# xiaoxiaokuye/CODLAD

Measured on NVIDIA B200. Metric: backmapped residues/sec (100-step, 10-ensemble), higher is better.
Workload: dtype f16 (tcgen05, fp32 accumulate)

## Files before the change

### codlad_b200/csrc/capi.cu

```cuda
#include <stdarg.h>
#include <string.h>

#include <map>
#include <string>
#include <vector>

#include "../../include/codlad_b200.h"
#include "decode.h"
#include "model.h"

namespace cb2 {

static thread_local char g_err[1024] = "";

void set_error(const char* fmt, ...) {
    va_list ap;
    va_start(ap, fmt);
    vsnprintf(g_err, sizeof(g_err), fmt, ap);
    va_end(ap);
}

float* plan_P(Plan& p, int which) { return p.P + (size_t)which * p.NB * p.L * 256; }

namespace {

struct TensorTable {
    std::map<std::string, const cb2_tensor*> by_name;
    TensorTable(const cb2_tensor* t, int n) {
        for (int i = 0; i < n; ++i) by_name[t[i].name] = &t[i];
    }
    const float* get(const std::string& name, long long numel) const {
        auto it = by_name.find(name);
        if (it == by_name.end()) { set_error("missing tensor '%s'", name.c_str()); return nullptr; }
        if (it->second->numel != numel) {
            set_error("tensor '%s': numel %lld, expected %lld", name.c_str(), it->second->numel, numel);
            return nullptr;
        }
        return it->second->data;
    }
};

struct Packer {
    std::vector<float> buf;
    size_t reserve(size_t n) {
        size_t off = (buf.size() + 63) & ~(size_t)63;
        buf.resize(off + n, 0.0f);
        return off;
    }
    size_t transposed(const float* W, int out, int in_total, int col0, int ncols, float scale = 1.0f) {
        size_t off = reserve((size_t)ncols * out);
        for (int k = 0; k < ncols; ++k)
            for (int o = 0; o < out; ++o) buf[off + (size_t)k * out + o] = scale * W[(size_t)o * in_total + col0 + k];
        return off;
    }
    size_t copy(const float* v, size_t n) {
        size_t off = reserve(n);
        memcpy(&buf[off], v, n * sizeof(float));
        return off;
    }
};

struct HalfPacker {
    std::vector<__half> buf;
    size_t block(const float* W, int in_total, int col0, float scale = 1.0f) {
        size_t off = buf.size();
        buf.resize(off + 128 * 128);
        for (int o = 0; o < 128; ++o)
            for (int k = 0; k < 128; ++k) buf[off + (size_t)o * 128 + k] = __float2half_rn(scale * W[(size_t)o * in_total + col0 + k]);
        return off;
    }
};

#define GET(var, name, numel)                               \
    const float* var = tt.get(name, (long long)(numel));    \
    if (!var) return 1;

template <typename T>
int dev_alloc(std::vector<void*>& owned, T** ptr, size_t count) {
    void* q = nullptr;
    CB2_CUDA(cudaMalloc(&q, count * sizeof(T) > 0 ? count * sizeof(T) : 16));
    owned.push_back(q);
    *ptr = reinterpret_cast<T*>(q);
    return 0;
}

}
}

using namespace cb2;

struct cb2_denoiser { DenoiserModel m; };
struct cb2_vae { VaeModel v; };
struct cb2_plan {
    Plan p;
    float* ca_full = nullptr;
    int *csr_row = nullptr, *csr_col = nullptr;
    int E = 0;
    signed char* orders = nullptr;
    int* slot_atom = nullptr;
    long long* out_off = nullptr;
    float *edge_w = nullptr, *S40 = nullptr, *phi = nullptr, *ic = nullptr, *zq = nullptr;
    int* vq_idx = nullptr;
    float *xa = nullptr, *xb = nullptr;
    int keep_debug = 0;
    bool frames_ready = false, topo_ready = false;
};

extern "C" {

int cb2_abi_version(void) { return CB2_ABI_VERSION; }
const char* cb2_last_error(void) { return cb2::g_err; }

int cb2_denoiser_create(const cb2_tensor* tensors, int n_tensors, const float* freqs128, int k_neighbors, cb2_denoiser** out) {
    if (!tensors || !freqs128 || !out) { set_error("denoiser_create: null argument"); return 1; }
    TensorTable tt(tensors, n_tensors);
    Packer pk;
    HalfPacker bp;
    const int H = CB2_H;
    std::map<std::string, size_t> off;
    std::map<std::string, size_t> boff;

    off["freqs"] = pk.copy(freqs128, 128);
    GET(te0w, "t_embedder.mlp.0.weight", H * 256) GET(te0b, "t_embedder.mlp.0.bias", H)
    GET(te2w, "t_embedder.mlp.2.weight", H * H) GET(te2b, "t_embedder.mlp.2.bias", H)
    off["te_w0_t"] = pk.transposed(te0w, H, 256, 0, 256); off["te_b0"] = pk.copy(te0b, H);
    off["te_w2_t"] = pk.transposed(te2w, H, H, 0, H); off["te_b2"] = pk.copy(te2b, H);

    {
        size_t wo = pk.reserve((size_t)H * CB2_MOD_TOTAL), bo = pk.reserve(CB2_MOD_TOTAL);
        off["ada_w_t"] = wo; off["ada_b"] = bo;
        int col = 0;
        auto put = [&](const std::string& pre, int width) -> int {
            const float* w = tt.get(pre + ".adaLN_modulation.1.weight", (long long)width * H);
            const float* b = tt.get(pre + ".adaLN_modulation.1.bias", width);
            if (!w || !b) return 1;
            for (int o = 0; o < width; ++o) {
                pk.buf[bo + col + o] = b[o];
                for (int k = 0; k < H; ++k) pk.buf[wo + (size_t)k * CB2_MOD_TOTAL + col + o] = w[(size_t)o * H + k];
            }
            col += width;
            return 0;
        };
        for (int l = 0; l < 3; ++l) if (put("encoder_layers." + std::to_string(l), CB2_MOD_ENC)) return 1;
        for (int l = 0; l < 3; ++l) if (put("decoder_layers." + std::to_string(l), CB2_MOD_DEC)) return 1;
        if (put("W_out", CB2_MOD_FIN)) return 1;
    }
    GET(xinw, "x_in.weight", H * 3) GET(xinb, "x_in.bias", H)
    off["xin_w_t"] = pk.transposed(xinw, H, 3, 0, 3); off["xin_b"] = pk.copy(xinb, H);

    GET(posw, "features.embeddings.linear.weight", 16 * 66) GET(posb, "features.embeddings.linear.bias", 16)
    GET(edgew, "features.edge_embedding.weight", H * 167)
    GET(lnw, "features.norm_edges.weight", H) GET(lnb, "features.norm_edges.bias", H)
    GET(wew, "W_e.weight", H * H) GET(web, "W_e.bias", H)
    {
        size_t o = pk.reserve(65 * H);
        for (int d = 0; d < 65; ++d)
            for (int c = 0; c < H; ++c) {
                double a = 0.0;
                for (int q = 0; q < 16; ++q) a += (double)(posw[q * 66 + d] + posb[q]) * (double)edgew[(size_t)c * 167 + q];
                pk.buf[o + (size_t)d * H + c] = (float)a;
            }
        off["pos_table"] = o;
        size_t w = pk.reserve(152 * H);
        for (int r = 0; r < 151; ++r)
            for (int c = 0; c < H; ++c) pk.buf[w + (size_t)r * H + c] = edgew[(size_t)c * 167 + 16 + r];
        off["wedge_t"] = w;
    }
    off["ln_w"] = pk.copy(lnw, H); off["ln_b"] = pk.copy(lnb, H);
    off["we_t"] = pk.transposed(wew, H, H, 0, H); off["we_b"] = pk.copy(web, H);

    GET(ws, "W_s.weight", 30 * H)
    for (int l = 0; l < 3; ++l) {
        const std::string p = "encoder_layers." + std::to_string(l), k = "e" + std::to_string(l) + ".";
        GET(w1, p + ".W1.weight", H * 3 * H) GET(b1, p + ".W1.bias", H) GET(w2, p + ".W2.weight", H * H) GET(b2, p + ".W2.bias", H)
        GET(w3, p + ".W3.weight", H * H) GET(b3, p + ".W3.bias", H)
        GET(w11, p + ".W11.weight", H * 3 * H) GET(b11, p + ".W11.bias", H) GET(w12, p + ".W12.weight", H * H) GET(b12, p + ".W12.bias", H)
        GET(w13, p + ".W13.weight", H * H) GET(b13, p + ".W13.bias", H)
        GET(win, p + ".dense.W_in.weight", 4 * H * H) GET(bin, p + ".dense.W_in.bias", 4 * H)
        GET(wout, p + ".dense.W_out.weight", H * 4 * H) GET(bout, p + ".dense.W_out.bias", H)
        off[k + "W1a_t"] = pk.transposed(w1, H, 3 * H, 0, H); off[k + "W1b_t"] = pk.transposed(w1, H, 3 * H, H, H);
        off[k + "W1c_t"] = pk.transposed(w1, H, 3 * H, 2 * H, H); off[k + "b1"] = pk.copy(b1, H);
        off[k + "W2_t"] = pk.transposed(w2, H, H, 0, H); off[k + "b2"] = pk.copy(b2, H);
        off[k + "W3_t"] = pk.transposed(w3, H, H, 0, H); off[k + "b3"] = pk.copy(b3, H);
        off[k + "W11a_t"] = pk.transposed(w11, H, 3 * H, 0, H); off[k + "W11b_t"] = pk.transposed(w11, H, 3 * H, H, H);
        off[k + "W11c_t"] = pk.transposed(w11, H, 3 * H, 2 * H, H); off[k + "b11"] = pk.copy(b11, H);
        off[k + "W12_t"] = pk.transposed(w12, H, H, 0, H); off[k + "b12"] = pk.copy(b12, H);
        off[k + "W13_t"] = pk.transposed(w13, H, H, 0, H); off[k + "b13"] = pk.copy(b13, H);
        off[k + "Win_t"] = pk.transposed(win, 4 * H, H, 0, H); off[k + "bin"] = pk.copy(bin, 4 * H);
        off[k + "Wout_t"] = pk.transposed(wout, H, 4 * H, 0, 4 * H); off[k + "bout"] = pk.copy(bout, H);
        boff[k + "W1b"] = bp.block(w1, 3 * H, H); boff[k + "W2"] = bp.block(w2, H, 0, 0.5f);
        boff[k + "W11b"] = bp.block(w11, 3 * H, H); boff[k + "W12"] = bp.block(w12, H, 0, 0.5f); boff[k + "W13"] = bp.block(w13, H, 0, 0.5f);
        boff[k + "W1a"] = bp.block(w1, 3 * H, 0); boff[k + "W1c"] = bp.block(w1, 3 * H, 2 * H);
        boff[k + "W11a"] = bp.block(w11, 3 * H, 0); boff[k + "W11c"] = bp.block(w11, 3 * H, 2 * H);
        boff[k + "W3"] = bp.block(w3, H, 0);
        for (int q = 0; q < 4; ++q) { size_t o = bp.block(win + (size_t)q * H * H, H, 0); if (q == 0) boff[k + "Win"] = o; }
        for (int q = 0; q < 4; ++q) { size_t o = bp.block(wout, 4 * H, q * H, 0.5f); if (q == 0) boff[k + "Wout"] = o; }
    }
    for (int l = 0; l < 3; ++l) {
        const std::string p = "decoder_layers." + std::to_string(l), k = "d" + std::to_string(l) + ".";
        GET(w1, p + ".W1.weight", H * 4 * H) GET(b1, p + ".W1.bias", H) GET(w2, p + ".W2.weight", H * H) GET(b2, p + ".W2.bias", H)
        GET(w3, p + ".W3.weight", H * H) GET(b3, p + ".W3.bias", H)
        GET(win, p + ".dense.W_in.weight", 4 * H * H) GET(bin, p + ".dense.W_in.bias", 4 * H)
        GET(wout, p + ".dense.W_out.weight", H * 4 * H) GET(bout, p + ".dense.W_out.bias", H)
        off[k + "W1a_t"] = pk.transposed(w1, H, 4 * H, 0, H); off[k + "W1b2_t"] = pk.transposed(w1, H, 4 * H, H, H, 2.0f);
        off[k + "W1d_t"] = pk.transposed(w1, H, 4 * H, 3 * H, H); off[k + "b1"] = pk.copy(b1, H);
        {
            size_t o = pk.reserve(30 * H);
            for (int z = 0; z < 30; ++z)
                for (int c = 0; c < H; ++c) {
                    double a = 0.0;
                    for (int q = 0; q < H; ++q) a += (double)ws[z * H + q] * (double)w1[(size_t)c * 4 * H + 2 * H + q];
                    pk.buf[o + (size_t)z * H + c] = (float)(2.0 * a);
                }
            off[k + "TS"] = o;
        }
        off[k + "W2_t"] = pk.transposed(w2, H, H, 0, H); off[k + "b2"] = pk.copy(b2, H);
        off[k + "W3_t"] = pk.transposed(w3, H, H, 0, H); off[k + "b3"] = pk.copy(b3, H);
        off[k + "Win_t"] = pk.transposed(win, 4 * H, H, 0, H); off[k + "bin"] = pk.copy(bin, 4 * H);
        off[k + "Wout_t"] = pk.transposed(wout, H, 4 * H, 0, 4 * H); off[k + "bout"] = pk.copy(bout, H);
        boff[k + "W1b2"] = bp.block(w1, 4 * H, H, 2.0f); boff[k + "W2"] = bp.block(w2, H, 0, 0.5f);
        boff[k + "W1a"] = bp.block(w1, 4 * H, 0); boff[k + "W1d"] = bp.block(w1, 4 * H, 3 * H);
        boff[k + "W3"] = bp.block(w3, H, 0);
        for (int q = 0; q < 4; ++q) { size_t o = bp.block(win + (size_t)q * H * H, H, 0); if (q == 0) boff[k + "Win"] = o; }
        for (int q = 0; q < 4; ++q) { size_t o = bp.block(wout, 4 * H, q * H, 0.5f); if (q == 0) boff[k + "Wout"] = o; }
    }
    GET(finw, "W_out.linear.weight", 6 * H) GET(finb, "W_out.linear.bias", 6)
    off["fin_w_t"] = pk.transposed(finw, 6, H, 0, H); off["fin_b"] = pk.copy(finb, 6);

    cb2_denoiser* d = new cb2_denoiser();
    DenoiserModel& m = d->m;
    m.k_neighbors = k_neighbors;
    CB2_CUDA(cudaMalloc(&m.dev_f32, pk.buf.size() * sizeof(float)));
    CB2_CUDA(cudaMemcpy(m.dev_f32, pk.buf.data(), pk.buf.size() * sizeof(float), cudaMemcpyHostToDevice));
    {
        std::vector<__half> v16;
        std::map<std::string, size_t> voff;
        auto putv = [&](const std::string& key, const float* src) {
            voff[key] = v16.size();
            for (int q = 0; q < H; ++q) v16.push_back(__float2half_rn(src[q]));
        };
        for (int l = 0; l < 3; ++l) {
            const std::string pe = "encoder_layers." + std::to_string(l), pd = "decoder_layers." + std::to_string(l);
            putv("e" + std::to_string(l) + ".b2", tt.get(pe + ".W2.bias", H));
            putv("e" + std::to_string(l) + ".b12", tt.get(pe + ".W12.bias", H));
            putv("e" + std::to_string(l) + ".b13", tt.get(pe + ".W13.bias", H));
            putv("d" + std::to_string(l) + ".b2", tt.get(pd + ".W2.bias", H));
        }
        CB2_CUDA(cudaMalloc(&m.dev_vec16, v16.size() * sizeof(__half)));
        CB2_CUDA(cudaMemcpy(m.dev_vec16, v16.data(), v16.size() * sizeof(__half), cudaMemcpyHostToDevice));
        for (int l = 0; l < 3; ++l) {
            m.enc[l].b2_16 = m.dev_vec16 + voff.at("e" + std::to_string(l) + ".b2");
            m.enc[l].b12_16 = m.dev_vec16 + voff.at("e" + std::to_string(l) + ".b12");
            m.enc[l].b13_16 = m.dev_vec16 + voff.at("e" + std::to_string(l) + ".b13");
            m.dec[l].b2_16 = m.dev_vec16 + voff.at("d" + std::to_string(l) + ".b2");
        }
    }
    CB2_CUDA(cudaMalloc(&m.dev_f16, bp.buf.size() * sizeof(__half)));
    CB2_CUDA(cudaMemcpy(m.dev_f16, bp.buf.data(), bp.buf.size() * sizeof(__half), cudaMemcpyHostToDevice));
    m.n_f16_blocks = (int)(bp.buf.size() / (128 * 128));
    auto F = [&](const std::string& key) { return (const float*)(m.dev_f32 + off.at(key)); };
    auto B = [&](const std::string& key) { return (const __half*)(m.dev_f16 + boff.at(key)); };
    m.freqs = F("freqs"); m.te_w0_t = F("te_w0_t"); m.te_b0 = F("te_b0"); m.te_w2_t = F("te_w2_t"); m.te_b2 = F("te_b2");
    m.ada_w_t = F("ada_w_t"); m.ada_b = F("ada_b"); m.xin_w_t = F("xin_w_t"); m.xin_b = F("xin_b");
    m.pos_table = F("pos_table"); m.wedge_t = F("wedge_t"); m.ln_w = F("ln_w"); m.ln_b = F("ln_b"); m.we_t = F("we_t"); m.we_b = F("we_b");
    for (int l = 0; l < 3; ++l) {
        const std::string k = "e" + std::to_string(l) + ".";
        EncLayerW& e = m.enc[l];
        e.W1a_t = F(k + "W1a_t"); e.W1b_t = F(k + "W1b_t"); e.W1c_t = F(k + "W1c_t"); e.b1 = F(k + "b1");
        e.W2_t = F(k + "W2_t"); e.b2 = F(k + "b2"); e.W3_t = F(k + "W3_t"); e.b3 = F(k + "b3");
        e.W11a_t = F(k + "W11a_t"); e.W11b_t = F(k + "W11b_t"); e.W11c_t = F(k + "W11c_t"); e.b11 = F(k + "b11");
        e.W12_t = F(k + "W12_t"); e.b12 = F(k + "b12"); e.W13_t = F(k + "W13_t"); e.b13 = F(k + "b13");
        e.Win_t = F(k + "Win_t"); e.bin = F(k + "bin"); e.Wout_t = F(k + "Wout_t"); e.bout = F(k + "bout");
        e.W1b_h = B(k + "W1b"); e.W2_h = B(k + "W2"); e.W11b_h = B(k + "W11b"); e.W12_h = B(k + "W12"); e.W13_h = B(k + "W13");
        e.W1a_h = B(k + "W1a"); e.W1c_h = B(k + "W1c"); e.W11a_h = B(k + "W11a"); e.W11c_h = B(k + "W11c");
        e.W3_h = B(k + "W3"); e.Win_h = B(k + "Win"); e.Wout_h = B(k + "Wout");
    }
    for (int l = 0; l < 3; ++l) {
        const std::string k = "d" + std::to_string(l) + ".";
        DecLayerW& e = m.dec[l];
        e.W1a_t = F(k + "W1a_t"); e.W1b2_t = F(k + "W1b2_t"); e.W1d_t = F(k + "W1d_t"); e.b1 = F(k + "b1"); e.TS = F(k + "TS");
        e.W2_t = F(k + "W2_t"); e.b2 = F(k + "b2"); e.W3_t = F(k + "W3_t"); e.b3 = F(k + "b3");
        e.Win_t = F(k + "Win_t"); e.bin = F(k + "bin"); e.Wout_t = F(k + "Wout_t"); e.bout = F(k + "bout");
        e.W1b2_h = B(k + "W1b2"); e.W2_h = B(k + "W2");
        e.W1a_h = B(k + "W1a"); e.W1d_h = B(k + "W1d"); e.W3_h = B(k + "W3"); e.Win_h = B(k + "Win"); e.Wout_h = B(k + "Wout");
    }
    m.fin_w_t = F("fin_w_t"); m.fin_b = F("fin_b");
    *out = d;
    return 0;
}

void cb2_denoiser_destroy(cb2_denoiser* d) {
    if (!d) return;
    cudaFree(d->m.dev_f32);
    cudaFree(d->m.dev_f16);
    cudaFree(d->m.dev_vec16);
    delete d;
}

int cb2_vae_create(const cb2_tensor* tensors, int n_tensors, const float* mean3, const float* std3, int angle_variant, cb2_vae** out) {
    if (!tensors || !mean3 || !std3 || !out) { set_error("vae_create: null argument"); return 1; }
    TensorTable tt(tensors, n_tensors);
    Packer pk;
    std::map<std::string, size_t> off;
    const std::string P = "equivaraintconv.";
    auto itcb = tt.by_name.find("quantize._codebook.embed");
    if (itcb == tt.by_name.end() || itcb->second->numel % 3 != 0) { set_error("missing/invalid quantize._codebook.embed"); return 1; }
    const int M = (int)(itcb->second->numel / 3);
    off["codebook"] = pk.copy(itcb->second->data, (size_t)M * 3);
    off["mean"] = pk.copy(mean3, 3); off["std"] = pk.copy(std3, 3);
    GET(mow, "map_out.weight", 36 * 3) GET(mob, "map_out.bias", 36)
    off["mapw_t"] = pk.transposed(mow, 36, 3, 0, 3); off["mapb"] = pk.copy(mob, 36);
    GET(remb, P + "res_embed.weight", 25 * 4) off["res_embed"] = pk.copy(remb, 100);
    const int D = 40, T = angle_variant ? 50 : 40;
    auto linear = [&](const std::string& key, const std::string& name, int o, int i) -> int {
        const float* w = tt.get(P + name + ".weight", (long long)o * i);
        const float* b = tt.get(P + name + ".bias", o);
        if (!w || !b) return 1;
        off[key + "_t"] = pk.transposed(w, o, i, 0, i);
        off[key + "_b"] = pk.copy(b, o);
        return 0;
    };
    size_t wd = pk.reserve(4 * 15 * D), bd = pk.reserve(4 * D);
    off["Wd_t"] = wd; off["bd"] = bd;
    for (int b = 0; b < 4; ++b) {
        const std::string s = std::to_string(b);
        if (linear("inv0." + s, "message_blocks." + s + ".inv_dense.0", D, D)) return 1;
        if (linear("inv1." + s, "message_blocks." + s + ".inv_dense.1", D, D)) return 1;
        GET(dw, P + "message_blocks." + s + ".dist_embed.block.1.weight", D * 15)
        GET(db, P + "message_blocks." + s + ".dist_embed.block.1.bias", D)
        for (int q = 0; q < 15; ++q)
            for (int c = 0; c < D; ++c) pk.buf[wd + ((size_t)b * 15 + q) * D + c] = dw[c * 15 + q];
        for (int c = 0; c < D; ++c) pk.buf[bd + b * D + c] = db[c];
        if (linear("db1." + s, "dense_blocks." + s + ".1", D, D)) return 1;
        if (linear("db3." + s, "dense_blocks." + s + ".3", D, D)) return 1;
        if (linear("tb1." + s, "sidechain_torsion_blocks." + s + ".1", T, T)) return 1;
        if (linear("tb3." + s, "sidechain_torsion_blocks." + s + ".3", T, T)) return 1;
    }
    GET(bbd, P + "backbone_dist.weight", 75) GET(scd, P + "sidechain_dist.weight", 250)
    off["bb_dist"] = pk.copy(bbd, 75); off["sc_dist"] = pk.copy(scd, 250);
    if (linear("ba1", "backbone_angle.1", 3, D) || linear("ba3", "backbone_angle.3", 3, 3)) return 1;
    if (linear("bt1", "backbone_torsion.1", 3, D + 3) || linear("bt3", "backbone_torsion.3", 3, 3)) return 1;
    if (angle_variant) {
        if (linear("sa1", "sidechain_angle.1", 10, D) || linear("sa3", "sidechain_angle.3", 10, 10)) return 1;
    } else {
        GET(sae, P + "sidechain_angle.weight", 250) off["sa_embed"] = pk.copy(sae, 250);
    }
    if (linear("ft1", "final_torsion.1", 10, T) || linear("ft3", "final_torsion.3", 10, 10)) return 1;

    cb2_vae* h = new cb2_vae();
    VaeModel& v = h->v;
    v.M = M; v.angle_variant = angle_variant;
    CB2_CUDA(cudaMalloc(&v.dev, pk.buf.size() * sizeof(float)));
    CB2_CUDA(cudaMemcpy(v.dev, pk.buf.data(), pk.buf.size() * sizeof(float), cudaMemcpyHostToDevice));
    auto F = [&](const std::string& key) -> const float* {
        auto it = off.find(key);
        return it == off.end() ? nullptr : (const float*)(v.dev + it->second);
    };
    v.codebook = F("codebook"); v.mean = F("mean"); v.stdv = F("std"); v.mapw_t = F("mapw_t"); v.mapb = F("mapb");
    v.res_embed = F("res_embed"); v.Wd_t = F("Wd_t"); v.bd = F("bd");
    for (int b = 0; b < 4; ++b) {
        const std::string s = std::to_string(b);
        v.inv0_t[b] = F("inv0." + s + "_t"); v.inv0_b[b] = F("inv0." + s + "_b");
        v.inv1_t[b] = F("inv1." + s + "_t"); v.inv1_b[b] = F("inv1." + s + "_b");
        v.db1_t[b] = F("db1." + s + "_t"); v.db1_b[b] = F("db1." + s + "_b");
        v.db3_t[b] = F("db3." + s + "_t"); v.db3_b[b] = F("db3." + s + "_b");
        v.tb1_t[b] = F("tb1." + s + "_t"); v.tb1_b[b] = F("tb1." + s + "_b");
        v.tb3_t[b] = F("tb3." + s + "_t"); v.tb3_b[b] = F("tb3." + s + "_b");
    }
    v.bb_dist = F("bb_dist"); v.sc_dist = F("sc_dist"); v.sa_embed = F("sa_embed");
    v.ba1_t = F("ba1_t"); v.ba1_b = F("ba1_b"); v.ba3_t = F("ba3_t"); v.ba3_b = F("ba3_b");
    v.bt1_t = F("bt1_t"); v.bt1_b = F("bt1_b"); v.bt3_t = F("bt3_t"); v.bt3_b = F("bt3_b");
    v.sa1_t = F("sa1_t"); v.sa1_b = F("sa1_b"); v.sa3_t = F("sa3_t"); v.sa3_b = F("sa3_b");
    v.ft1_t = F("ft1_t"); v.ft1_b = F("ft1_b"); v.ft3_t = F("ft3_t"); v.ft3_b = F("ft3_b");
    CB2_CUDA(cudaMalloc(&v.e2, (size_t)M * sizeof(float)));
    if (int e = launch_codebook_norms(v.codebook, M, v.e2, 0)) return e;
    CB2_CUDA(cudaStreamSynchronize(0));
    *out = h;
    return 0;
}

void cb2_vae_destroy(cb2_vae* h) {
    if (!h) return;
    cudaFree(h->v.dev);
    cudaFree(h->v.e2);
    delete h;
}

int cb2_plan_create(const cb2_denoiser* d, int F, int NB, int L, int precision, int keep_debug, cb2_plan** out) {
    if (!out || F <= 0 || NB <= 0 || L <= 0) { set_error("plan_create: bad argument"); return 1; }
    if (precision != PREC_F32 && precision != PREC_F16) { set_error("plan_create: unknown precision %d", precision); return 1; }
    cb2_plan* h = new cb2_plan();
    Plan& p = h->p;
    p.model = d ? &d->m : nullptr; p.F = F; p.NB = NB; p.L = L; p.precision = precision;
    h->keep_debug = keep_debug;
    if (!d) {
        int e = 0;
        e |= dev_alloc(p.allocs, &p.X, (size_t)F * L * 3);
        e |= dev_alloc(p.allocs, &p.lengths, F);
        e |= dev_alloc(p.allocs, &p.cg_z, (size_t)F * L);
        e |= dev_alloc(p.allocs, &p.frame_of, NB);
        if (e) { cb2_plan_destroy(h); return e; }
        *out = h;
        return 0;
    }
    p.K = d->m.k_neighbors < L ? d->m.k_neighbors : L;
    const size_t N = (size_t)NB * L, FE = (size_t)F * L * p.K, NE = N * p.K;
    const size_t esz = precision == PREC_F16 ? 2 : 4;
    int e = 0;
    e |= dev_alloc(p.allocs, &p.X, (size_t)F * L * 3);
    e |= dev_alloc(p.allocs, &p.lengths, F);
    e |= dev_alloc(p.allocs, &p.cg_z, (size_t)F * L);
    e |= dev_alloc(p.allocs, &p.frame_of, NB);
    e |= dev_alloc(p.allocs, &p.nbr_idx, FE);
    e |= dev_alloc(p.allocs, &p.nbr_dist, FE);
    e |= dev_alloc(p.allocs, reinterpret_cast<unsigned char**>(&p.hE0), FE * 128 * esz);
    e |= dev_alloc(p.allocs, reinterpret_cast<unsigned char**>(&p.hE), NE * 128 * esz);
    if (keep_debug) e |= dev_alloc(p.allocs, &p.E_dbg, FE * 128);
    e |= dev_alloc(p.allocs, &p.hV, N * 128);
    e |= dev_alloc(p.allocs, &p.hVenc, N * 128);
    e |= dev_alloc(p.allocs, &p.P, 2 * N * 256);
    if (precision == PREC_F16) {
        e |= dev_alloc(p.allocs, &p.P16[0], N * 256);
        e |= dev_alloc(p.allocs, &p.P16[1], N * 256);
    }
    e |= dev_alloc(p.allocs, &p.S, N * 128);
    e |= dev_alloc(p.allocs, &p.out6, N * 6);
    e |= dev_alloc(p.allocs, &h->xa, N * 3);
    e |= dev_alloc(p.allocs, &h->xb, N * 3);
    p.mod_capacity = NB > 1024 ? NB : 1024;
    e |= dev_alloc(p.allocs, &p.mod, (size_t)p.mod_capacity * CB2_MOD_TOTAL);
    if (precision == PREC_F16) e |= dev_alloc(p.allocs, &p.mod16, (size_t)p.mod_capacity * 768);
    e |= dev_alloc(p.allocs, &p.silu_c, (size_t)p.mod_capacity * 128);
    e |= dev_alloc(p.allocs, &p.tvals, p.mod_capacity);
    e |= dev_alloc(p.allocs, &p.coef, (size_t)p.mod_capacity * 8);
    if (e) { cb2_plan_destroy(h); return e; }
    if (precision == PREC_F16) {
        if (int r = edge_tc_prepare(p)) { cb2_plan_destroy(h); return r; }
        if (int r = node_tc_prepare(p)) { cb2_plan_destroy(h); return r; }
    }
    *out = h;
    return 0;
}

void cb2_plan_destroy(cb2_plan* h) {
    if (!h) return;
    if (h->p.graph) cudaGraphExecDestroy(h->p.graph);
    edge_tc_release(h->p);
    node_tc_release(h->p);
    for (void* q : h->p.allocs) cudaFree(q);
    delete h;
}

int cb2_plan_K(const cb2_plan* h) { return h ? h->p.K : 0; }
long long cb2_plan_launches(const cb2_plan* h) { return h ? h->p.launches : 0; }

int cb2_plan_set_frames(cb2_plan* h, const float* X, const int* lengths, const int* cg_z, const int* frame_of, void* stream) {
    if (!h || !X || !lengths || !cg_z || !frame_of) { set_error("set_frames: null argument"); return 1; }
    Plan& p = h->p;
    cudaStream_t s = (cudaStream_t)stream;
    CB2_CUDA(cudaMemcpyAsync(p.X, X, (size_t)p.F * p.L * 3 * sizeof(float), cudaMemcpyDeviceToDevice, s));
    CB2_CUDA(cudaMemcpyAsync(p.lengths, lengths, p.F * sizeof(int), cudaMemcpyDeviceToDevice, s));
    CB2_CUDA(cudaMemcpyAsync(p.cg_z, cg_z, (size_t)p.F * p.L * sizeof(int), cudaMemcpyDeviceToDevice, s));
    CB2_CUDA(cudaMemcpyAsync(p.frame_of, frame_of, p.NB * sizeof(int), cudaMemcpyDeviceToDevice, s));
    if (p.model == nullptr) { h->frames_ready = true; return 0; }
    {
        std::vector<int> len((size_t)p.F);
        CB2_CUDA(cudaMemcpyAsync(len.data(), p.lengths, (size_t)p.F * sizeof(int), cudaMemcpyDeviceToHost, s));
        CB2_CUDA(cudaStreamSynchronize(s));
        p.all_full = true;
        for (int f = 0; f < p.F; ++f) p.all_full = p.all_full && len[f] >= p.L;
    }
    if (int e = launch_knn(p.X, p.lengths, p.F, p.L, p.K, p.nbr_dist, p.nbr_idx, s)) return e;
    if (int e = launch_edge_features(*p.model, p.X, p.lengths, p.nbr_idx, p.nbr_dist, p.F, p.L, p.K, p.E_dbg, p.hE0, p.precision, s)) return e;
    p.launches += 2;
    h->frames_ready = true;
    return 0;
}

}

namespace {

int edge_dispatch(Plan& p, int mode, int layer, const float* mod_base, int mod_stride, cudaStream_t s) {
    return p.precision == PREC_F16 ? launch_edge_tc(p, mode, layer, mod_base, mod_stride, s)
                                    : launch_edge_f32(p, mode, layer, mod_base, mod_stride, s);
}

int run_forward(Plan& p, const float* x, const float* mod_base, int mod_stride, const float* noise, float* x_next,
                const float* coef_row, const float* inpaint_row, cudaStream_t s, int stop_after = -1) {
    int n = 0;
    auto done = [&]() { return stop_after >= 0 && ++n >= stop_after; };
    const bool tc = p.precision == PREC_F16 && p.node_tc != nullptr;
    auto node_update = [&](int phase, const float* xt, const float* nz, float* xn, const float* cf, const float* iq) {
        return tc ? launch_node_update_tc(p, phase, mod_base, mod_stride, xt, nz, xn, cf, iq, s)
                  : launch_node_update(p, phase, mod_base, mod_stride, xt, nz, xn, cf, iq, s);
    };
    if (int e = tc ? launch_node_init_tc(p, x, s) : launch_node_init(p, x, mod_base, mod_stride, s)) return e;
    if (done()) return 0;
    for (int l = 0; l < 3; ++l) {
        if (int e = edge_dispatch(p, EDGE_ENC_NODE, l, mod_base, mod_stride, s)) return e;
        if (done()) return 0;
        if (int e = node_update(l, nullptr, nullptr, nullptr, nullptr, nullptr)) return e;
        if (done()) return 0;
        if (int e = edge_dispatch(p, EDGE_ENC_EDGE, l, mod_base, mod_stride, s)) return e;
        if (done()) return 0;
    }
    for (int l = 0; l < 3; ++l) {
        if (int e = edge_dispatch(p, EDGE_DEC, l, mod_base, mod_stride, s)) return e;
        if (done()) return 0;
        const bool last = l == 2;
        if (int e = node_update(3 + l, last ? x : nullptr, last ? noise : nullptr, last ? x_next : nullptr, last ? coef_row : nullptr,
                                last ? inpaint_row : nullptr)) return e;
        if (done()) return 0;
    }
    return 0;
}

}

extern "C" {

int cb2_plan_forward_partial(cb2_plan* h, const float* x, const float* t, int stop_after, void* stream) {
    if (!h || !x || !t) { set_error("forward_partial: null argument"); return 1; }
    if (!h->frames_ready || !h->p.model) { set_error("forward_partial: no denoiser frames on this plan"); return 1; }
    Plan& p = h->p;
    cudaStream_t s = (cudaStream_t)stream;
    if (int e = launch_timestep_mod(*p.model, t, p.NB, p.silu_c, p.mod, p.mod16, s)) return e;
    p.coef_steps = 0;
    return run_forward(p, x, p.mod, CB2_MOD_TOTAL, nullptr, nullptr, nullptr, nullptr, s, stop_after);
}

int cb2_plan_forward(cb2_plan* h, const float* x, const float* t, float* out, void* stream) {
    if (!h || !x || !t || !out) { set_error("forward: null argument"); return 1; }
    if (!h->frames_ready || !h->p.model) { set_error("forward: cb2_plan_set_frames has not been called (or decode-only plan)"); return 1; }
    Plan& p = h->p;
    cudaStream_t s = (cudaStream_t)stream;
    if (p.NB > p.mod_capacity) { set_error("forward: NB exceeds table capacity"); return 1; }
    if (int e = launch_timestep_mod(*p.model, t, p.NB, p.silu_c, p.mod, p.mod16, s)) return e;
    p.launches += 2;
    p.coef_steps = 0;
    if (int e = run_forward(p, x, p.mod, CB2_MOD_TOTAL, nullptr, nullptr, nullptr, nullptr, s)) return e;
    CB2_CUDA(cudaMemcpyAsync(out, p.out6, (size_t)p.NB * p.L * 6 * sizeof(float), cudaMemcpyDeviceToDevice, s));
    return 0;
}

static int set_schedule(cb2_plan* h, const float* t_of_step, const float* coef, int T, int kind, cudaStream_t s) {
    if (!h || !t_of_step || !coef || T <= 0 || !h->p.model) { set_error("set_schedule: bad argument"); return 1; }
    Plan& p = h->p;
    if (T > p.mod_capacity) { set_error("set_schedule: T=%d exceeds capacity %d", T, p.mod_capacity); return 1; }
    CB2_CUDA(cudaMemcpyAsync(p.tvals, t_of_step, T * sizeof(float), cudaMemcpyHostToDevice, s));
    CB2_CUDA(cudaMemcpyAsync(p.coef, coef, (size_t)T * 8 * sizeof(float), cudaMemcpyHostToDevice, s));
    if (int e = launch_timestep_mod(*p.model, p.tvals, T, p.silu_c, p.mod, p.mod16, s)) return e;
    CB2_CUDA(cudaStreamSynchronize(s));
    p.launches += 2;
    p.coef_steps = T;
    p.update_kind = kind;
    p.coef_noisy = kind == UPDATE_DDPM;
    for (int i = 0; i < T && !p.coef_noisy; ++i) p.coef_noisy = coef[(size_t)i * 8 + 4] != 0.0f;
    if (p.graph) { cudaGraphExecDestroy(p.graph); p.graph = nullptr; }
    return 0;
}

int cb2_plan_set_schedule(cb2_plan* h, const float* t_of_step, const float* coef, int T, void* stream) {
    return set_schedule(h, t_of_step, coef, T, UPDATE_DDPM, (cudaStream_t)stream);
}

int cb2_plan_set_ddim_schedule(cb2_plan* h, const float* t_of_step, const float* ddim_coef, int T, void* stream) {
    return set_schedule(h, t_of_step, ddim_coef, T, UPDATE_DDIM, (cudaStream_t)stream);
}

int cb2_plan_set_inpaint(cb2_plan* h, const unsigned char* keep, const float* x0, const float* q_coef, int T, void* stream) {
    if (!h || !h->p.model) { set_error("set_inpaint: bad argument"); return 1; }
    Plan& p = h->p;
    if (!keep) { p.inpaint = false; return 0; }
    if (!x0 || !q_coef || T <= 0) { set_error("set_inpaint: x0, q_coef and T > 0 are required with a keep mask"); return 1; }
    if (T > p.mod_capacity) { set_error("set_inpaint: T=%d exceeds capacity %d", T, p.mod_capacity); return 1; }
    cudaStream_t s = (cudaStream_t)stream;
    const size_t N = (size_t)p.NB * p.L;
    if (!p.inp_keep) {
        unsigned char* keep_buf = nullptr;
        float *x0_buf = nullptr, *eps_buf = nullptr, *coef_buf = nullptr;
        int e = 0;
        e |= dev_alloc(p.allocs, &keep_buf, N);
        e |= dev_alloc(p.allocs, &x0_buf, N * 3);
        e |= dev_alloc(p.allocs, &eps_buf, N * 3);
        e |= dev_alloc(p.allocs, &coef_buf, (size_t)(p.mod_capacity + 1) * 2);
        if (e) return e;
        p.inp_keep = keep_buf; p.inp_x0 = x0_buf; p.inp_eps = eps_buf; p.inp_coef = coef_buf;
    }
    CB2_CUDA(cudaMemcpyAsync(p.inp_keep, keep, N, cudaMemcpyDeviceToDevice, s));
    CB2_CUDA(cudaMemcpyAsync(p.inp_x0, x0, N * 3 * sizeof(float), cudaMemcpyDeviceToDevice, s));
    const size_t nq = (size_t)(T + 1) * 2;
    if (p.inp_coef_host.size() != nq || memcmp(p.inp_coef_host.data(), q_coef, nq * sizeof(float)) != 0) {
        p.inp_coef_host.assign(q_coef, q_coef + nq);
        CB2_CUDA(cudaMemcpyAsync(p.inp_coef, q_coef, nq * sizeof(float), cudaMemcpyHostToDevice, s));
        CB2_CUDA(cudaStreamSynchronize(s));
    }
    p.inpaint_steps = T;
    p.inpaint = true;
    return 0;
}

static int enqueue_loop(cb2_plan* h, float* x, const float* noise, cudaStream_t s) {
    Plan& p = h->p;
    const size_t n3 = (size_t)p.NB * p.L * 3;
    CB2_CUDA(cudaMemcpyAsync(h->xa, x, n3 * sizeof(float), cudaMemcpyDeviceToDevice, s));
    if (p.inpaint) {
        if (int e = launch_inpaint_init(p.inp_keep, p.inp_x0, p.inp_coef + (size_t)p.coef_steps * 2, p.NB * p.L, h->xa, p.inp_eps, s)) return e;
        p.launches++;
    }
    float *cur = h->xa, *nxt = h->xb;
    for (int step = p.coef_steps - 1; step >= 0; --step) {
        const float* mod_row = p.mod + (size_t)step * CB2_MOD_TOTAL;
        const float* step_noise = noise != nullptr ? noise + (size_t)step * n3 : nullptr;
        const float* inpaint_row = p.inpaint ? p.inp_coef + (size_t)step * 2 : nullptr;
        if (int e = run_forward(p, cur, mod_row, 0, step_noise, nxt, p.coef + (size_t)step * 8, inpaint_row, s)) {
            char prev[1024];
            snprintf(prev, sizeof(prev), "%s", g_err);
            const unsigned int* tl = edge_tc_trap_log();
            if (tl != nullptr) {
                char w[600]; int n = 0;
                for (int i = 0; i < 18 && n < 560; ++i)
                    if (tl[4 + 2 * i]) n += snprintf(w + n, sizeof(w) - n, " w%d:bar+0x%x/p%u", i, tl[4 + 2 * i] & 0xfffu, tl[5 + 2 * i] >> 16);
                set_error("%s [sampling step %d; block %u timed-out waits:%s]", prev, step, tl[0] - 1u, w);
            }
            else set_error("%s [sampling step %d]", prev, step);
            return e;
        }
        float* t = cur; cur = nxt; nxt = t;
    }
    CB2_CUDA(cudaMemcpyAsync(x, cur, n3 * sizeof(float), cudaMemcpyDeviceToDevice, s));
    return 0;
}

int cb2_plan_sample(cb2_plan* h, float* x, const float* noise, int use_graph, void* stream) {
    if (!h || !x) { set_error("sample: null argument"); return 1; }
    Plan& p = h->p;
    if (!h->frames_ready || p.coef_steps <= 0) { set_error("sample: set_frames / set_schedule must be called first"); return 1; }
    if (!noise && p.coef_noisy) { set_error("sample: noise may be NULL only on a DDIM schedule whose sigma are all zero (eta = 0)"); return 1; }
    if (p.inpaint && p.inpaint_steps != p.coef_steps) {
        set_error("sample: the inpainting table has T=%d, the schedule T=%d", p.inpaint_steps, p.coef_steps);
        return 1;
    }
    cudaStream_t s = (cudaStream_t)stream;
    if (!use_graph) return enqueue_loop(h, x, noise, s);
    if (!p.graph || p.graph_key[0] != x || p.graph_key[1] != noise || p.graph_steps != p.coef_steps || p.graph_all_full != p.all_full ||
        p.graph_inpaint != p.inpaint) {
        if (p.graph) { cudaGraphExecDestroy(p.graph); p.graph = nullptr; }
        cudaStream_t cs;
        CB2_CUDA(cudaStreamCreateWithFlags(&cs, cudaStreamNonBlocking));
        const long long before = p.launches;
        CB2_CUDA(cudaStreamBeginCapture(cs, cudaStreamCaptureModeThreadLocal));
        int e = enqueue_loop(h, x, noise, cs);
        cudaGraph_t g = nullptr;
        cudaError_t ce = cudaStreamEndCapture(cs, &g);
        p.launches = before;
        if (e || ce != cudaSuccess) {
            if (g) cudaGraphDestroy(g);
            cudaStreamDestroy(cs);
            if (!e) set_error("graph capture failed: %s", cudaGetErrorString(ce));
            return e ? e : (int)ce;
        }
        ce = cudaGraphInstantiate(&p.graph, g, 0);
        cudaGraphDestroy(g);
        cudaStreamDestroy(cs);
        if (ce != cudaSuccess) { set_error("graph instantiate failed: %s", cudaGetErrorString(ce)); p.graph = nullptr; return (int)ce; }
        p.graph_key[0] = x; p.graph_key[1] = noise; p.graph_steps = p.coef_steps; p.graph_all_full = p.all_full;
        p.graph_inpaint = p.inpaint;
    }
    CB2_CUDA(cudaGraphLaunch(p.graph, s));
    p.launches += 16LL * p.coef_steps + (p.inpaint ? 1 : 0);
    return 0;
}

int cb2_plan_set_topology(cb2_plan* h, const cb2_vae* v, const float* ca_full, const int* csr_row_ptr, const int* csr_col,
                          int n_edges, const signed char* atom_orders, const int* slot_atom, const long long* out_offset,
                          void* stream) {
    if (!h || !v || !ca_full || !csr_row_ptr || !atom_orders || !slot_atom || !out_offset) { set_error("set_topology: null argument"); return 1; }
    Plan& p = h->p;
    cudaStream_t s = (cudaStream_t)stream;
    const size_t N = (size_t)p.NB * p.L, FL = (size_t)p.F * p.L;
    if (!h->ca_full) {
        int e = 0;
        e |= dev_alloc(p.allocs, &h->ca_full, (size_t)p.F * (p.L + 2) * 3);
        e |= dev_alloc(p.allocs, &h->csr_row, FL + 1);
        e |= dev_alloc(p.allocs, &h->orders, FL * 30);
        e |= dev_alloc(p.allocs, &h->slot_atom, FL * 14);
        e |= dev_alloc(p.allocs, &h->out_off, p.NB);
        e |= dev_alloc(p.allocs, &h->S40, N * 40);
        e |= dev_alloc(p.allocs, &h->phi, N * 40);
        e |= dev_alloc(p.allocs, &h->ic, N * 39);
        e |= dev_alloc(p.allocs, &h->zq, N * 3);
        e |= dev_alloc(p.allocs, &h->vq_idx, N);
        if (e) return e;
    }
    if (n_edges > h->E || !h->csr_col) {
        int e = dev_alloc(p.allocs, &h->csr_col, (size_t)n_edges);
        e |= dev_alloc(p.allocs, &h->edge_w, (size_t)4 * n_edges * 40);
        if (e) return e;
    }
    h->E = n_edges;
    CB2_CUDA(cudaMemcpyAsync(h->ca_full, ca_full, (size_t)p.F * (p.L + 2) * 3 * sizeof(float), cudaMemcpyDeviceToDevice, s));
    CB2_CUDA(cudaMemcpyAsync(h->csr_row, csr_row_ptr, (FL + 1) * sizeof(int), cudaMemcpyDefault, s));
    if (n_edges) CB2_CUDA(cudaMemcpyAsync(h->csr_col, csr_col, (size_t)n_edges * sizeof(int), cudaMemcpyDefault, s));
    CB2_CUDA(cudaMemcpyAsync(h->orders, atom_orders, FL * 30, cudaMemcpyDefault, s));
    CB2_CUDA(cudaMemcpyAsync(h->slot_atom, slot_atom, FL * 14 * sizeof(int), cudaMemcpyDefault, s));
    CB2_CUDA(cudaMemcpyAsync(h->out_off, out_offset, p.NB * sizeof(long long), cudaMemcpyDefault, s));
    if (!h->frames_ready) { set_error("set_topology: call cb2_plan_set_frames first (needs X)"); return 1; }
    if (int e = launch_ic_edge_filters(v->v, p.X, p.F, p.L, h->csr_row, h->csr_col, n_edges, h->edge_w, s)) return e;
    p.launches += 1;
    CB2_CUDA(cudaStreamSynchronize(s));
    h->topo_ready = true;
    return 0;
}

int cb2_plan_decode(cb2_plan* h, const cb2_vae* v, const float* latent, int denorm, int* idx, float* zq, float* ic_recon,
                    float* xyz, void* stream) {
    if (!h || !v || !latent) { set_error("decode: null argument"); return 1; }
    if (!h->topo_ready) { set_error("decode: cb2_plan_set_topology has not been called"); return 1; }
    Plan& p = h->p;
    cudaStream_t s = (cudaStream_t)stream;
    const int N = p.NB * p.L;
    if (int e = launch_vq_lookup(v->v, latent, N, p.L, p.lengths, p.frame_of, denorm, h->vq_idx, h->zq, h->S40, s)) return e;
    if (int e = launch_ic_decoder(v->v, h->S40, h->phi, N, p.L, p.frame_of, p.lengths, p.cg_z, h->csr_row, h->csr_col, h->E,
                                  h->edge_w, h->ic, s, &p.launches)) return e;
    p.launches += 1;
    if (idx) CB2_CUDA(cudaMemcpyAsync(idx, h->vq_idx, (size_t)N * sizeof(int), cudaMemcpyDeviceToDevice, s));
    if (zq) CB2_CUDA(cudaMemcpyAsync(zq, h->zq, (size_t)N * 3 * sizeof(float), cudaMemcpyDeviceToDevice, s));
    if (ic_recon) CB2_CUDA(cudaMemcpyAsync(ic_recon, h->ic, (size_t)N * 39 * sizeof(float), cudaMemcpyDeviceToDevice, s));
    if (xyz) {
        if (int e = launch_ic_to_xyz(h->ca_full, h->ic, N, p.L, p.frame_of, p.lengths, h->orders, h->slot_atom, h->out_off, xyz,
                                     nullptr, s)) return e;
        p.launches += 1;
    }
    return 0;
}

int cb2_plan_buffer(cb2_plan* h, const char* name, void* dst, long long dst_bytes, void* stream) {
    if (!h || !name || !dst) { set_error("plan_buffer: null argument"); return 1; }
    void* src = nullptr;
    long long size = 0;
    void** ptr = &src;
    long long* bytes = &size;
    Plan& p = h->p;
    const size_t N = (size_t)p.NB * p.L, FE = (size_t)p.F * p.L * p.K, esz = p.precision == PREC_F16 ? 2 : 4;
    const std::string n = name;
    if (n == "nbr_idx") { *ptr = p.nbr_idx; *bytes = FE * 4; }
    else if (n == "nbr_dist") { *ptr = p.nbr_dist; *bytes = FE * 4; }
    else if (n == "E") { *ptr = p.E_dbg; *bytes = p.E_dbg ? FE * 128 * 4 : 0; }
    else if (n == "hE0") { *ptr = p.hE0; *bytes = FE * 128 * esz; }
    else if (n == "hE") { *ptr = p.hE; *bytes = N * p.K * 128 * esz; }
    else if (n == "hV") { *ptr = p.hV; *bytes = N * 128 * 4; }
    else if (n == "S") { *ptr = p.S; *bytes = N * 128 * 4; }
    else if (n == "out6") { *ptr = p.out6; *bytes = N * 6 * 4; }
    else if (n == "tc_trace") {
        if (!p.tc_trace) { unsigned long long* t = nullptr; if (dev_alloc(p.allocs, &t, 6144)) return 1; cudaMemsetAsync(t, 0, 49152, (cudaStream_t)stream); p.tc_trace = t; }
        *ptr = p.tc_trace; *bytes = 49152;
    }
    else if (n == "mod") { *ptr = p.mod; *bytes = (size_t)p.mod_capacity * CB2_MOD_TOTAL * 4; }
    else { set_error("plan_buffer: unknown buffer '%s'", name); return 1; }
    if (!src || dst_bytes > size) { set_error("plan_buffer: '%s' holds %lld bytes, %lld requested", name, size, dst_bytes); return 1; }
    CB2_CUDA(cudaMemcpyAsync(dst, src, (size_t)dst_bytes, cudaMemcpyDeviceToDevice, (cudaStream_t)stream));
    return 0;
}

int cb2_plan_run_edge_kernel(cb2_plan* h, int mode, int layer, void* stream) {
    if (!h || mode < 0 || mode > 2 || layer < 0 || layer > 2) { set_error("run_edge_kernel: bad argument"); return 1; }
    if (!h->frames_ready || h->p.coef_steps <= 0) { set_error("run_edge_kernel: set_frames / set_schedule first"); return 1; }
    return edge_dispatch(h->p, mode, layer, h->p.mod, 0, (cudaStream_t)stream);
}

int cb2_plan_run_stage(cb2_plan* h, const cb2_vae* v, int stage, int layer, float* xyz_scratch, void* stream) {
    if (!h || stage < 0 || stage > 9) { set_error("run_stage: bad argument"); return 1; }
    Plan& p = h->p;
    cudaStream_t s = (cudaStream_t)stream;
    if (!h->frames_ready) { set_error("run_stage: set_frames first"); return 1; }
    if (stage <= 3 && (p.coef_steps <= 0 || !p.model)) { set_error("run_stage: set_schedule first"); return 1; }
    if (stage >= 6 && (!h->topo_ready || !v)) { set_error("run_stage: set_topology first (and pass the vae)"); return 1; }
    const int N = p.NB * p.L;
    switch (stage) {
        case 0: case 1: case 2:
            if (layer < 0 || layer > 2) { set_error("run_stage: layer"); return 1; }
            return edge_dispatch(p, stage, layer, p.mod, 0, s);
        case 3: {
            if (layer < 0 || layer > 5) { set_error("run_stage: phase"); return 1; }
            const bool last = layer == 5, tc = p.precision == PREC_F16 && p.node_tc != nullptr;
            const float *xt = last ? h->xa : nullptr, *nz = last ? h->xa : nullptr, *cf = last ? p.coef : nullptr;
            float* xn = last ? h->xb : nullptr;
            return tc ? launch_node_update_tc(p, layer, p.mod, 0, xt, nz, xn, cf, nullptr, s)
                      : launch_node_update(p, layer, p.mod, 0, xt, nz, xn, cf, nullptr, s);
        }
        case 4: return launch_knn(p.X, p.lengths, p.F, p.L, p.K, p.nbr_dist, p.nbr_idx, s);
        case 5: return launch_edge_features(*p.model, p.X, p.lengths, p.nbr_idx, p.nbr_dist, p.F, p.L, p.K, p.E_dbg, p.hE0, p.precision, s);
        case 6: return launch_vq_lookup(v->v, h->xa, N, p.L, p.lengths, p.frame_of, 1, h->vq_idx, h->zq, h->S40, s);
        case 7: return launch_ic_decoder(v->v, h->S40, h->phi, N, p.L, p.frame_of, p.lengths, p.cg_z, h->csr_row, h->csr_col, h->E, h->edge_w, h->ic, s, &p.launches);
        case 8:
            if (!xyz_scratch) { set_error("run_stage: ic_to_xyz needs xyz_scratch"); return 1; }
            return launch_ic_to_xyz(h->ca_full, h->ic, N, p.L, p.frame_of, p.lengths, h->orders, h->slot_atom, h->out_off, xyz_scratch, nullptr, s);
        default: return launch_ic_edge_filters(v->v, p.X, p.F, p.L, h->csr_row, h->csr_col, h->E, h->edge_w, s);
    }
}

int cb2_knn_topk(const float* X, const int* lengths, int F, int L, int K, float* D, int* idx, void* stream) {
    if (!X || !D || !idx) { set_error("knn_topk: null argument"); return 1; }
    return launch_knn(X, lengths, F, L, K, D, idx, (cudaStream_t)stream);
}

int cb2_vq_lookup(const cb2_vae* v, const float* x, int NB, int L, const int* lengths, const int* frame_of, int denorm,
                  int* idx, float* zq, void* stream) {
    if (!v || !x || !lengths || !frame_of || !idx || !zq) { set_error("vq_lookup: null argument"); return 1; }
    return launch_vq_lookup(v->v, x, NB * L, L, lengths, frame_of, denorm, idx, zq, nullptr, (cudaStream_t)stream);
}

int cb2_p_sample(const float* x, const float* model_out, const float* noise, const float* coef, const int* step_of_member,
                 int rows_per_member, int rows, int C, float* x_next, void* stream) {
    if (!x || !model_out || !noise || !coef || !step_of_member || !x_next) { set_error("p_sample: null argument"); return 1; }
    return launch_p_sample(x, model_out, noise, coef, step_of_member, rows_per_member, rows, C, x_next, (cudaStream_t)stream);
}

int cb2_ddim_sample(const float* x, const float* model_out, const float* noise, const float* coef, const int* step_of_member,
                    int rows_per_member, int rows, int C, float* x_next, void* stream) {
    if (!x || !model_out || !coef || !step_of_member || !x_next) { set_error("ddim_sample: null argument"); return 1; }
    return launch_ddim_sample(x, model_out, noise, coef, step_of_member, rows_per_member, rows, C, x_next, (cudaStream_t)stream);
}

int cb2_ic_to_xyz(const float* ca_full, const float* ic_recon, int NB, int L, const int* frame_of, const int* lengths,
                  const signed char* atom_orders, const int* slot_atom, const long long* out_offset, float* xyz, void* stream) {
    if (!ca_full || !ic_recon || !frame_of || !lengths || !atom_orders || !slot_atom || !out_offset || !xyz) {
        set_error("ic_to_xyz: null argument");
        return 1;
    }
    return launch_ic_to_xyz(ca_full, ic_recon, NB * L, L, frame_of, lengths, atom_orders, slot_atom, out_offset, xyz, nullptr,
                            (cudaStream_t)stream);
}

}
```

### codlad_b200/csrc/model.h

```cpp
#pragma once
#include <cuda_runtime.h>
#include <cuda_fp16.h>
#include <stdint.h>
#include <string>
#include <unordered_map>
#include <vector>

#include "common.cuh"

namespace cb2 {

struct EncLayerW {
    const float *W1a_t, *W1b_t, *W1c_t, *b1, *W2_t, *b2, *W3_t, *b3;
    const float *W11a_t, *W11b_t, *W11c_t, *b11, *W12_t, *b12, *W13_t, *b13;
    const float *Win_t, *bin, *Wout_t, *bout;
    const __half *W1b_h, *W2_h, *W11b_h, *W12_h, *W13_h;
    const __half *W1a_h, *W1c_h, *W11a_h, *W11c_h, *W3_h, *Win_h , *Wout_h ;
    const __half *b2_16, *b12_16, *b13_16;
};

struct DecLayerW {
    const float *W1a_t, *W1b2_t , *W1d_t, *b1, *TS ;
    const float *W2_t, *b2, *W3_t, *b3, *Win_t, *bin, *Wout_t, *bout;
    const __half *W1b2_h, *W2_h;
    const __half *W1a_h, *W1d_h, *W3_h, *Win_h , *Wout_h ;
    const __half* b2_16;
};

struct DenoiserModel {
    int k_neighbors = 64;
    int vocab = 30;
    const float *freqs , *te_w0_t, *te_b0, *te_w2_t, *te_b2, *ada_w_t, *ada_b;
    const float *xin_w_t , *xin_b;
    const float *pos_table, *wedge_t, *ln_w, *ln_b, *we_t, *we_b;
    EncLayerW enc[3];
    DecLayerW dec[3];
    const float *fin_w_t , *fin_b;
    float* dev_f32 = nullptr;
    __half* dev_f16 = nullptr;
    __half* dev_vec16 = nullptr;
    int n_f16_blocks = 0;
};

enum Precision { PREC_F32 = 0, PREC_F16 = 1 };
enum UpdateKind { UPDATE_DDPM = 0, UPDATE_DDIM = 1 };

struct Plan {
    const DenoiserModel* model = nullptr;
    int F = 0, NB = 0, L = 0, K = 0, precision = PREC_F32;
    int T_rows = 0;
    float* X = nullptr;
    int* lengths = nullptr;
    int* cg_z = nullptr;
    int* frame_of = nullptr;
    int* nbr_idx = nullptr;
    float* nbr_dist = nullptr;
    void* hE0 = nullptr;
    float* E_dbg = nullptr;
    void* hE = nullptr;
    float* hV = nullptr;
    float* hVenc = nullptr;
    float* P = nullptr;
    __half* P16[2] = {nullptr, nullptr};
    __half* mod16 = nullptr;
    int num_sms = 148;
    bool all_full = false;
    unsigned long long* tc_trace = nullptr;
    float* silu_c = nullptr;
    float* S = nullptr;
    float* out6 = nullptr;
    float* mod = nullptr;
    int mod_capacity = 0;
    int* mod_row = nullptr;
    float* tvals = nullptr;
    float* coef = nullptr;
    int coef_steps = 0;
    int update_kind = 0;
    bool coef_noisy = true;
    bool inpaint = false;
    int inpaint_steps = 0;
    unsigned char* inp_keep = nullptr;
    float* inp_x0 = nullptr;
    float* inp_eps = nullptr;
    float* inp_coef = nullptr;
    std::vector<float> inp_coef_host;
    cudaGraphExec_t graph = nullptr;
    const void* graph_key[4] = {nullptr, nullptr, nullptr, nullptr};
    int graph_steps = 0;
    bool graph_all_full = false;
    bool graph_inpaint = false;
    std::vector<void*> allocs;
    void* tmaps = nullptr;
    void* node_tc = nullptr;
    long long launches = 0;
};

int launch_knn(const float* X, const int* lengths, int F, int L, int K, float* D, int* idx, cudaStream_t s);
int launch_edge_features(const DenoiserModel& m, const float* X, const int* lengths, const int* idx, const float* D,
                         int F, int L, int K, float* E_dbg, void* hE0, int precision, cudaStream_t s);
int launch_edge_raw_features(const float* X, const int* idx, const float* D, int F, int L, int K, float* raw_out, cudaStream_t s);
int launch_timestep_mod(const DenoiserModel& m, const float* tvals, int n, float* scratch_silu_c, float* mod, __half* mod16, cudaStream_t s);
int launch_p_sample(const float* x, const float* out6, const float* noise, const float* coef_rows, const int* step_of_row,
                    int rows_per_b, int n_rows, int C, float* x_next, cudaStream_t s);
int launch_ddim_sample(const float* x, const float* out6, const float* noise, const float* coef_rows, const int* step_of_row,
                       int rows_per_b, int n_rows, int C, float* x_next, cudaStream_t s);
int launch_inpaint_init(const unsigned char* keep, const float* x0, const float* q_head, int n_rows, float* x, float* eps, cudaStream_t s);
float* plan_P(Plan& p, int which);

struct NodeArgs;
int launch_node_init(Plan& p, const float* x, const float* mod_base, int mod_stride_b, cudaStream_t s);
int launch_node_update(Plan& p, int phase , const float* mod_base, int mod_stride_b,
                       const float* x_t, const float* noise, float* x_next, const float* coef_row, const float* inpaint_row,
                       cudaStream_t s);
int launch_edge_f32(Plan& p, int mode, int layer, const float* mod_base, int mod_stride_b, cudaStream_t s);
int launch_edge_tc(Plan& p, int mode, int layer, const float* mod_base, int mod_stride_b, cudaStream_t s);
int edge_tc_prepare(Plan& p);
int node_tc_prepare(Plan& p);
void node_tc_release(Plan& p);
int launch_node_init_tc(Plan& p, const float* x, cudaStream_t s);
int launch_node_update_tc(Plan& p, int phase, const float* mod_base, int mod_stride_b, const float* x_t, const float* noise,
                          float* x_next, const float* coef_row, const float* inpaint_row, cudaStream_t s);
void edge_tc_release(Plan& p);
const unsigned int* edge_tc_trap_log();

enum EdgeMode { EDGE_ENC_NODE = 0, EDGE_ENC_EDGE = 1, EDGE_DEC = 2 };

}
```

### codlad_b200/csrc/node_tc.cu

```cuda
#include "node_tc_body.cuh"

namespace cb2 {

using namespace tc;

namespace {

template <bool INPAINT>
__device__ __forceinline__ void node_tc_run(const CUtensorMap& wmap, const NodeTcParams& p, const InpaintRows& ir) {
    extern __shared__ __align__(1024) unsigned char smem[];
    __shared__ uint32_t s_tmem;
    const int tid = threadIdx.x, warp = tid >> 5;
    if (tid == 0) trace_window(p.trace, p.trace_slot, false);
    if ((smem_u32(smem) & 1023u) != 0) __trap();
    pdl_launch_dependents();
    if (warp == 16) {
        asm volatile("tcgen05.alloc.cta_group::1.sync.aligned.shared::cta.b32 [%0], 512;" ::"r"(smem_u32(&s_tmem)) : "memory");
        asm volatile("tcgen05.relinquish_alloc_permit.cta_group::1.sync.aligned;" ::: "memory");
    }
    tc_fence_before();
    __syncthreads();
    tc_fence_after();
    const uint32_t tmem_base = s_tmem;
    node_block<INPAINT>(smem, tmem_base, &wmap, p, blockIdx.x * NT, p.N, true, ir);
    if (tid == 0) trace_window(p.trace, p.trace_slot, true);
    if (warp == 16) asm volatile("tcgen05.dealloc.cta_group::1.sync.aligned.b32 %0, 512;" ::"r"(tmem_base) : "memory");
}

__global__ void __launch_bounds__(NODE_CTA_THREADS, 1) node_tc_kernel(const __grid_constant__ CUtensorMap wmap, const NodeTcParams p) {
    node_tc_run<false>(wmap, p, InpaintRows{});
}

__global__ void __launch_bounds__(NODE_CTA_THREADS, 1) node_tc_inpaint_kernel(const __grid_constant__ CUtensorMap wmap, const NodeTcParams p,
                                                                             const __grid_constant__ InpaintRows ir) {
    node_tc_run<true>(wmap, p, ir);
}


struct NodeTcState { CUtensorMap wmap; };

int node_tc_launch(Plan& p, NodeTcParams& np, cudaStream_t s, const InpaintRows* ir = nullptr) {
    const NodeTcState& st = *reinterpret_cast<const NodeTcState*>(p.node_tc);
    const dim3 grid((np.N + NT - 1) / NT), block(NODE_CTA_THREADS);
    if (ir != nullptr) CB2_CUDA(launch_pdl(node_tc_inpaint_kernel, grid, block, NODE_TC_SMEM, s, st.wmap, np, *ir));
    else CB2_CUDA(launch_pdl(node_tc_kernel, grid, block, NODE_TC_SMEM, s, st.wmap, np));
    CB2_LAUNCH_CHECK();
    p.launches++;
    return 0;
}

void base_params(Plan& p, NodeTcParams& np) {
    np = NodeTcParams{};
    np.N = p.NB * p.L; np.L = p.L; np.K = p.K;
    np.lengths = p.lengths; np.frame_of = p.frame_of; np.nbr_idx = p.nbr_idx; np.cg_z = p.cg_z;
    np.hV = p.hV; np.hVenc = p.hVenc; np.S = p.S;
    np.trace = p.tc_trace; np.trace_slot = p.launches & 2047;
}

}

int node_tc_prepare(Plan& p) {
    EncodeTiledFn fn = nullptr;
    if (get_encode_fn(&fn)) return 1;
    NodeTcState* st = new NodeTcState();
    p.node_tc = st;
    if (encode_rows_map(fn, &st->wmap, p.model->dev_f16, (size_t)p.model->n_f16_blocks * 128, 128)) return 1;
    CB2_CUDA(cudaFuncSetAttribute(node_tc_kernel, cudaFuncAttributeMaxDynamicSharedMemorySize, (int)NODE_TC_SMEM));
    CB2_CUDA(cudaFuncSetAttribute(node_tc_inpaint_kernel, cudaFuncAttributeMaxDynamicSharedMemorySize, (int)NODE_TC_SMEM));
    return 0;
}

void node_tc_release(Plan& p) {
    delete reinterpret_cast<NodeTcState*>(p.node_tc);
    p.node_tc = nullptr;
}

int launch_node_init_tc(Plan& p, const float* x, cudaStream_t s) {
    const DenoiserModel& m = *p.model;
    auto row_of = [&](const __half* w) { return (int)((w - m.dev_f16) / 128); };
    NodeTcParams np;
    base_params(p, np);
    np.do_update = 0;
    np.x = x; np.xin_w_t = m.xin_w_t; np.xin_b = m.xin_b;
    np.n_proj = 1;
    np.proj[0] = ProjTc{row_of(m.enc[0].W1a_h), row_of(m.enc[0].W1c_h), m.enc[0].b1, nullptr, p.P16[0], 0};
    return node_tc_launch(p, np, s);
}

void node_tc_update_params(Plan& p, int phase, const float* mod_base, int mod_stride_b, const float* x_t, const float* noise,
                           float* x_next, const float* coef_row, tc::NodeTcParams& np) {
    const DenoiserModel& m = *p.model;
    auto row_of = [&](const __half* w) { return (int)((w - m.dev_f16) / 128); };
    base_params(p, np);
    np.do_update = 1;
    np.mod_stride = mod_stride_b;
    if (phase < 3) {
        const EncLayerW& e = m.enc[phase];
        np.masked_count = 1;
        np.w3_row = row_of(e.W3_h); np.win_row = row_of(e.Win_h); np.wout_row = row_of(e.Wout_h);
        np.b3 = e.b3; np.bin = e.bin; np.bout = e.bout;
        np.mod = mod_base + CB2_MOD_ENC_OFF(phase);
        np.n_proj = 2;
        np.proj[0] = ProjTc{row_of(e.W11a_h), row_of(e.W11c_h), e.b11, nullptr, p.P16[1], 0};
        if (phase < 2) {
            const EncLayerW& nx = m.enc[phase + 1];
            np.proj[1] = ProjTc{row_of(nx.W1a_h), row_of(nx.W1c_h), nx.b1, nullptr, p.P16[0], 0};
        } else {
            const DecLayerW& d = m.dec[0];
            np.write_enc = 1;
            np.proj[1] = ProjTc{row_of(d.W1a_h), row_of(d.W1d_h), d.b1, d.TS, p.P16[0], 2};
        }
    } else {
        const int l = phase - 3;
        const DecLayerW& d = m.dec[l];
        np.masked_count = 0;
        np.w3_row = row_of(d.W3_h); np.win_row = row_of(d.Win_h); np.wout_row = row_of(d.Wout_h);
        np.b3 = d.b3; np.bin = d.bin; np.bout = d.bout;
        np.mod = mod_base + CB2_MOD_DEC_OFF(l);
        if (l < 2) {
            const DecLayerW& nx = m.dec[l + 1];
            np.n_proj = 1;
            np.proj[0] = ProjTc{row_of(nx.W1a_h), row_of(nx.W1d_h), nx.b1, nx.TS, p.P16[0], 1};
        } else {
            np.n_proj = 0;
            np.do_final = 1;
            np.fin_mod = mod_base + CB2_MOD_FIN_OFF;
            np.fin_w_t = m.fin_w_t; np.fin_b = m.fin_b;
            np.out6 = p.out6;
            np.x_t = x_t; np.noise = noise; np.x_next = x_next; np.coef = coef_row;
            np.ddim = p.update_kind == UPDATE_DDIM;
        }
    }
}

int launch_node_update_tc(Plan& p, int phase, const float* mod_base, int mod_stride_b, const float* x_t, const float* noise,
                          float* x_next, const float* coef_row, const float* inpaint_row, cudaStream_t s) {
    NodeTcParams np;
    node_tc_update_params(p, phase, mod_base, mod_stride_b, x_t, noise, x_next, coef_row, np);
    if (inpaint_row != nullptr && np.do_final) {
        const InpaintRows ir{p.inp_keep, p.inp_x0, p.inp_eps, inpaint_row};
        return node_tc_launch(p, np, s, &ir);
    }
    return node_tc_launch(p, np, s);
}

}
```

### codlad_b200/csrc/node_tc_body.cuh

```cuda
#pragma once
#include "model.h"
#include "tc_common.cuh"

namespace cb2 {
namespace tc {

struct ProjTc {
    int wa_row, wc_row;
    const float *ba, *table;
    __half* out16;
    int add_enc;
};

struct NodeTcParams {
    int N, L, K;
    int do_update, masked_count;
    const float *x, *xin_w_t, *xin_b;
    const float* S;
    int w3_row, win_row, wout_row;
    const float *b3, *bin, *bout;
    const float* mod;
    int mod_stride;
    const int *lengths, *frame_of, *nbr_idx, *cg_z;
    float *hV, *hVenc;
    int write_enc;
    ProjTc proj[2];
    int n_proj;
    int do_final;
    const float *fin_mod, *fin_w_t, *fin_b;
    float* out6;
    const float *x_t, *noise, *coef;
    float* x_next;
    int ddim;
    unsigned long long* trace;
    int trace_slot;
};

constexpr int NODE_EPI_THREADS = 512;
constexpr int NODE_CTA_THREADS = NODE_EPI_THREADS + 64;
constexpr int NT = 32;
constexpr int NPTH = NT / 4;
constexpr int ACT_HALF = NT * 128;
constexpr int ACT_BYTES = 2 * ACT_HALF;
constexpr int N_SLOT = 5;
constexpr int N_ACT = 6;
constexpr int MAX_WT = 13;
constexpr int R1 = 0, R2 = NT, R3 = 5 * NT;
static_assert(NT == 32, "the LayerNorm transpose-reduce below is written for 8 nodes per thread");

__device__ __forceinline__ void node_epi_sync() { asm volatile("bar.sync 1, 512;" ::: "memory"); }
__device__ __forceinline__ void node_group_sync(int cq) { asm volatile("bar.sync %0, 128;" ::"r"(cq + 2) : "memory"); }

__device__ __forceinline__ uint32_t act_off(int r, int f) {
    return (uint32_t)((f >> 6) * ACT_HALF + r * 128 + ((((f >> 3) & 7) ^ (r & 7)) << 4) + (f & 7) * 2);
}
__device__ __forceinline__ void sts_h(unsigned char* p, __half h) { *reinterpret_cast<__half*>(p) = h; }

__device__ __forceinline__ int weight_rows(const NodeTcParams& p, int* rows) {
    int n = 0;
    if (p.do_update) {
        rows[n++] = p.w3_row;
        for (int c = 0; c < 4; ++c) rows[n++] = p.win_row + 128 * c;
        for (int c = 0; c < 4; ++c) rows[n++] = p.wout_row + 128 * c;
    }
    for (int j = 0; j < p.n_proj; ++j) { rows[n++] = p.proj[j].wa_row; rows[n++] = p.proj[j].wc_row; }
    return n;
}

constexpr int N_BAR = 20;
constexpr size_t NODE_TC_SMEM = (size_t)N_SLOT * TILE_BYTES + (size_t)N_ACT * ACT_BYTES + 2 * 4 * 4 * 16 * 4 + 4 * NT * 4 + N_BAR * 8 + 16;

template <bool INPAINT>
__device__ __forceinline__ void node_block(unsigned char* smem, const uint32_t tmem_base, const CUtensorMap* wmap_p, const NodeTcParams& p,
                                           const int node0, const int n_end, const bool dep_wait, const InpaintRows& ir) {
    unsigned char* sW = smem;
    unsigned char* sAct = sW + N_SLOT * TILE_BYTES;
    float* sRed = reinterpret_cast<float*>(sAct + N_ACT * ACT_BYTES);
    int* sB = reinterpret_cast<int*>(sRed + 2 * 4 * 4 * 16);
    float* sMk = reinterpret_cast<float*>(sB + NT);
    float* sCnt = sMk + NT;
    int* sZ = reinterpret_cast<int*>(sCnt + NT);
    uint64_t* sBar = reinterpret_cast<uint64_t*>(sZ + NT);

    const int tid = threadIdx.x, warp = tid >> 5, lane = tid & 31;
    auto bar_full = [&](int s) { return smem_u32(&sBar[s]); };
    auto bar_free = [&](int s) { return smem_u32(&sBar[N_SLOT + s]); };
    const uint32_t bar_mma = smem_u32(&sBar[10]), bar_act = smem_u32(&sBar[11]);
    auto bar_chunk = [&](int c) { return smem_u32(&sBar[12 + c]); };
    auto bar_mid = [&](int c) { return smem_u32(&sBar[16 + c]); };
    if (tid == 0) {
        for (int s = 0; s < N_SLOT; ++s) { mbar_init(bar_full(s), 1); mbar_init(bar_free(s), 1); }
        mbar_init(bar_mma, 1); mbar_init(bar_act, NODE_EPI_THREADS / 32);
        for (int c = 0; c < 4; ++c) { mbar_init(bar_chunk(c), 1); mbar_init(bar_mid(c), NODE_EPI_THREADS / 32); }
        asm volatile("fence.mbarrier_init.release.cluster;" ::: "memory");
    }
    if (tid < NT) {
        const int n = min(node0 + tid, n_end - 1);
        const int b = n / p.L, i = n - b * p.L;
        const int f = __ldg(p.frame_of + b);
        const int len = __ldg(p.lengths + f);
        float cnt = (float)p.K;
        if (p.masked_count && len < p.L) {
            int cn = 0;
            if (i < len) {
                const int* row = p.nbr_idx + ((size_t)f * p.L + i) * p.K;
                for (int k = 0; k < p.K; ++k) cn += __ldg(row + k) < len ? 1 : 0;
            }
            cnt = (float)cn;
        }
        sB[tid] = b; sMk[tid] = i < len ? 1.f : 0.f; sCnt[tid] = cnt; sZ[tid] = __ldg(p.cg_z + (size_t)f * p.L + i);
    }
    tc_fence_before();
    __syncthreads();
    tc_fence_after();
    constexpr uint32_t IDESC = umma_idesc(128, NT, 0, 0);
    auto act_tile = [&](int t) { return sAct + t * ACT_BYTES; };

    if (warp >= 16) {
        if (warp == 17) {
            int rows[MAX_WT];
            const int nt = weight_rows(p, rows);
            for (int i = 0; i < nt; ++i) {
                const int slot = i % N_SLOT, use = i / N_SLOT;
                if (use > 0) mbar_wait(bar_free(slot), (uint32_t)((use - 1) & 1));
                if (elect_one()) {
                    mbar_expect_tx(bar_full(slot), (uint32_t)TILE_BYTES);
                    for (int h = 0; h < 2; ++h)
                        tma_load_2d(smem_u32(sW + slot * TILE_BYTES + h * HALF_BYTES), wmap_p, h * 64, rows[i], bar_full(slot));
                }
                __syncwarp();
            }
        } else if (warp == 16) {
#ifdef CB2_TRACE_CTRL
            unsigned long long* ctrace = (p.trace != nullptr && blockIdx.x == 0 && lane == 0) ? p.trace + 512 : nullptr;
            int n_ct = 0;
            auto cmark = [&](int ev) {
                if (ctrace != nullptr && n_ct < 400) {
                    unsigned long long t;
                    asm volatile("mov.u64 %0, %%globaltimer;" : "=l"(t));
                    ctrace[1 + n_ct] = (t << 8) | (unsigned long long)ev;
                    ctrace[0] = (unsigned long long)(++n_ct);
                }
            };
#else
            auto cmark = [](int) {};
#endif
            cmark(0);
            uint32_t ph_act = 0;
            int ti = 0;
            auto gemm = [&](int act, int d_col, bool accumulate) {
                const int slot = ti % N_SLOT;
                mbar_wait(bar_full(slot), (uint32_t)((ti / N_SLOT) & 1));
                tc_fence_after();
                cmark(6);
                const uint64_t a0 = umma_desc(smem_u32(sW + slot * TILE_BYTES), 16, 1024), b0 = umma_desc(smem_u32(act_tile(act)), 16, 1024);
                if (elect_one()) {
#pragma unroll
                    for (int k = 0; k < 8; ++k)
                        umma_f16(tmem_base + (uint32_t)d_col, a0 + (uint64_t)(((k >> 2) * HALF_BYTES + (k & 3) * 32) >> 4),
                                 b0 + (uint64_t)(((k >> 2) * ACT_HALF + (k & 3) * 32) >> 4), IDESC, (accumulate || k > 0) ? 1u : 0u);
                    umma_commit(bar_free(slot));
                }
                __syncwarp();
                cmark(7);
                ++ti;
            };
            auto commit_phase = [&]() { if (elect_one()) umma_commit(bar_mma); __syncwarp(); cmark(4); };
            auto wait_act = [&]() { mbar_wait(bar_act, ph_act); ph_act ^= 1; tc_fence_after(); cmark(2); };
            if (p.do_update) {
                wait_act(); gemm(0, R1, false); commit_phase();
                wait_act();
                for (int c = 0; c < 4; ++c) { gemm(1, R2 + c * NT, false); if (elect_one()) umma_commit(bar_chunk(c)); __syncwarp(); }
                for (int c = 0; c < 4; ++c) { mbar_wait(bar_mid(c), 0); tc_fence_after(); cmark(8); gemm(2 + c, R3, c > 0); }
                commit_phase();
            }
            if (p.n_proj > 0) {
                wait_act();
                for (int j = 0; j < p.n_proj; ++j) {
                    gemm(0, R2 + (2 * j) * NT, false);
                    gemm(p.proj[j].add_enc ? 1 : 0, R2 + (2 * j + 1) * NT, false);
                }
                commit_phase();
            }
        }
    } else {
        const int quarter = warp & 3, cq = warp >> 2;
        const int fl = quarter * 32 + lane;
        const int nl0 = cq * NPTH;
        const uint32_t tmem_lane = tmem_base + ((uint32_t)(quarter * 32) << 16) + (uint32_t)nl0;
        uint32_t ph_mma = 0;
        int red_use = 0;
        float v[NPTH];
        auto publish = [&]() { fence_async_smem(); tc_fence_before(); __syncwarp(); if (lane == 0) mbar_arrive(bar_act); };
        auto wait_mma = [&]() { mbar_wait(bar_mma, ph_mma); ph_mma ^= 1; tc_fence_after(); };
        auto live = [&](int i) { return node0 + nl0 + i < n_end; };
        auto gnode = [&](int i) { return (size_t)(node0 + nl0 + i); };
        auto store_act = [&](unsigned char* tile, const float* x) {
#pragma unroll
            for (int i = 0; i < NPTH; ++i) sts_h(tile + act_off(nl0 + i, fl), __float2half_rn(x[i]));
        };
        auto node_stats = [&](float* mean, float* rstd) {
            float q[16];
#pragma unroll
            for (int i = 0; i < 8; ++i) { q[i] = v[i]; q[8 + i] = v[i] * v[i]; }
#pragma unroll
            for (int cnt = 8, off = 16; cnt >= 1; cnt >>= 1, off >>= 1) {
                const bool upper = (lane & off) != 0;
#pragma unroll
                for (int j = 0; j < cnt; ++j) {
                    const float send = upper ? q[j] : q[j + cnt];
                    const float keep = upper ? q[j + cnt] : q[j];
                    q[j] = keep + __shfl_xor_sync(0xffffffffu, send, off);
                }
            }
            q[0] += __shfl_xor_sync(0xffffffffu, q[0], 1);
            const int idx = ((lane >> 4) & 1) * 8 + ((lane >> 3) & 1) * 4 + ((lane >> 2) & 1) * 2 + ((lane >> 1) & 1);
            float* red = sRed + ((red_use & 1) * 16 + cq * 4) * 16;
            if ((lane & 1) == 0) red[quarter * 16 + idx] = q[0];
            node_group_sync(cq);
            float tot[16];
#pragma unroll
            for (int k4 = 0; k4 < 4; ++k4) {
                const float4 a = *reinterpret_cast<const float4*>(red + 0 * 16 + k4 * 4), b = *reinterpret_cast<const float4*>(red + 1 * 16 + k4 * 4);
                const float4 c = *reinterpret_cast<const float4*>(red + 2 * 16 + k4 * 4), d = *reinterpret_cast<const float4*>(red + 3 * 16 + k4 * 4);
                tot[k4 * 4] = (a.x + b.x) + (c.x + d.x); tot[k4 * 4 + 1] = (a.y + b.y) + (c.y + d.y);
                tot[k4 * 4 + 2] = (a.z + b.z) + (c.z + d.z); tot[k4 * 4 + 3] = (a.w + b.w) + (c.w + d.w);
            }
#pragma unroll
            for (int i = 0; i < 8; ++i) {
                mean[i] = tot[i] * (1.0f / 128.0f);
                rstd[i] = rsqrtf(fmaxf(tot[8 + i] * (1.0f / 128.0f) - mean[i] * mean[i], 0.f) + 1e-6f);
            }
            ++red_use;
        };
        const int b_first = sB[nl0], b_last = sB[nl0 + NPTH - 1];
        struct ModRow { float sh, sc, gt; };
        auto fetch_mod = [&](const float* mod_sh) {
            const float* m = mod_sh + (size_t)b_first * p.mod_stride + fl;
            return ModRow{__ldg(m), __ldg(m + 128), __ldg(m + 256)};
        };
        auto modulate = [&](const float* mod_sh, const ModRow& mr, bool masked) {
            float mean[8], rstd[8];
            node_stats(mean, rstd);
            float A = mr.gt * (1.0f + mr.sc), Bv = mr.gt * mr.sh;
#pragma unroll
            for (int i = 0; i < 8; ++i) {
                if (b_first != b_last) {
                    const float* m = mod_sh + (size_t)sB[nl0 + i] * p.mod_stride + fl;
                    const float sh = __ldg(m), sc = __ldg(m + 128), gt = __ldg(m + 256);
                    A = gt * (1.0f + sc); Bv = gt * sh;
                }
                const float t = fmaf((v[i] - mean[i]) * rstd[i], A, Bv);
                v[i] = masked ? sMk[nl0 + i] * t : t;
            }
        };

        const int enc_mode = p.n_proj > 0 ? p.proj[p.n_proj - 1].add_enc : 0;
        float pj_ba[2] = {0.f, 0.f}, pj_tab[NPTH], h_enc[NPTH];
        int tab_j = -1;
#pragma unroll
        for (int i = 0; i < NPTH; ++i) { pj_tab[i] = 0.f; h_enc[i] = 0.f; }
#pragma unroll
        for (int j = 0; j < 2; ++j) {
            if (j < p.n_proj) {
                pj_ba[j] = __ldg(p.proj[j].ba + fl);
                if (p.proj[j].table != nullptr) {
                    tab_j = j;
#pragma unroll
                    for (int i = 0; i < NPTH; ++i) pj_tab[i] = __ldg(p.proj[j].table + sZ[nl0 + i] * 128 + fl);
                }
            }
        }
        if (dep_wait) pdl_wait();
        if (enc_mode == 1) {
#pragma unroll
            for (int i = 0; i < NPTH; ++i) h_enc[i] = live(i) ? p.hVenc[gnode(i) * 128 + fl] : 0.f;
        }
        if (p.do_update) {
            {
                const int node = tid >> 4, c16 = tid & 15;
                uint32_t o[4] = {0u, 0u, 0u, 0u};
                if (node0 + node < n_end) {
                    uint32_t r8[8];
                    ldg256_coherent(p.S + (size_t)(node0 + node) * 128 + c16 * 8, r8);
#pragma unroll
                    for (int e = 0; e < 4; ++e) o[e] = f2_to_h2(__uint_as_float(r8[2 * e]), __uint_as_float(r8[2 * e + 1]));
                }
                *reinterpret_cast<uint4*>(act_tile(0) + (c16 >> 3) * ACT_HALF + node * 128 + (((c16 & 7) ^ (node & 7)) << 4)) = make_uint4(o[0], o[1], o[2], o[3]);
            }
#pragma unroll
            for (int i = 0; i < NPTH; ++i) v[i] = live(i) ? p.hV[gnode(i) * 128 + fl] : 0.f;
            publish();
            {
                const float b3 = __ldg(p.b3 + fl);
                const ModRow mr = fetch_mod(p.mod);
                wait_mma();
                float acc[8];
                tmem_ld8(tmem_lane + R1, acc);
#pragma unroll
                for (int i = 0; i < NPTH; ++i) v[i] += (acc[i] + sCnt[nl0 + i] * b3) * (1.0f / 30.0f);
                modulate(p.mod, mr, false);
                store_act(act_tile(1), v);
            }
            publish();
            {
                float bi[4];
#pragma unroll
                for (int c = 0; c < 4; ++c) bi[c] = __ldg(p.bin + c * 128 + fl);
#pragma unroll
                for (int c = 0; c < 4; ++c) {
                    mbar_wait(bar_chunk(c), 0);
                    tc_fence_after();
                    float acc[8];
                    tmem_ld8(tmem_lane + (uint32_t)(R2 + c * NT), acc);
                    unsigned char* dst = act_tile(2 + c);
#pragma unroll
                    for (int j = 0; j < 4; ++j) {
                        const __half2 g = gelu2_h2(as_h2(pack_sat(acc[2 * j] + bi[c], acc[2 * j + 1] + bi[c])));
                        sts_h(dst + act_off(nl0 + 2 * j, fl), __low2half(g));
                        sts_h(dst + act_off(nl0 + 2 * j + 1, fl), __high2half(g));
                    }
                    fence_async_smem(); tc_fence_before(); __syncwarp();
                    if (lane == 0) mbar_arrive(bar_mid(c));
                }
            }
            {
                const float bo = __ldg(p.bout + fl);
                const ModRow mr = fetch_mod(p.mod + 384);
                wait_mma();
                float acc[8];
                tmem_ld8(tmem_lane + R3, acc);
#pragma unroll
                for (int i = 0; i < NPTH; ++i) v[i] += acc[i] + bo;
                modulate(p.mod + 384, mr, true);
            }
        } else {
            const float w0 = __ldg(p.xin_w_t + fl), w1 = __ldg(p.xin_w_t + 128 + fl), w2 = __ldg(p.xin_w_t + 256 + fl), bb = __ldg(p.xin_b + fl);
#pragma unroll
            for (int i = 0; i < NPTH; ++i) {
                v[i] = 0.f;
                if (live(i)) {
                    const float* x = p.x + gnode(i) * 3;
                    v[i] = fmaf(x[2], w2, fmaf(x[1], w1, fmaf(x[0], w0, bb)));
                }
            }
        }
        auto write_state = [&]() {
#pragma unroll
            for (int i = 0; i < NPTH; ++i) {
                if (live(i)) {
                    p.hV[gnode(i) * 128 + fl] = v[i];
                    if (p.write_enc) p.hVenc[gnode(i) * 128 + fl] = v[i];
                }
            }
        };
        if (p.n_proj == 0) write_state();
        if (p.n_proj > 0) {
            store_act(act_tile(0), v);
            if (enc_mode) {
                float hp[NPTH];
#pragma unroll
                for (int i = 0; i < NPTH; ++i)
                    hp[i] = enc_mode == 1 ? (live(i) ? v[i] + h_enc[i] : 0.f) : 2.0f * v[i];
                store_act(act_tile(1), hp);
            }
            publish();
            write_state();
            wait_mma();
            for (int j = 0; j < p.n_proj; ++j) {
                const ProjTc pj = p.proj[j];
#pragma unroll
                for (int which = 0; which < 2; ++which) {
                    float acc[8];
                    tmem_ld8(tmem_lane + (uint32_t)(R2 + (2 * j + which) * NT), acc);
#pragma unroll
                    for (int i = 0; i < NPTH; ++i) {
                        if (live(i)) {
                            const float add = which == 0 ? (j == 0 ? pj_ba[0] : pj_ba[1]) : (j == tab_j ? pj_tab[i] : 0.f);
                            pj.out16[gnode(i) * 256 + which * 128 + fl] = __float2half_rn(acc[i] + add);
                        }
                    }
                }
            }
        }
        if (p.do_final) {
            float* sH = reinterpret_cast<float*>(act_tile(2));
#pragma unroll
            for (int i = 0; i < NPTH; ++i) sH[(nl0 + i) * 128 + fl] = v[i];
            node_epi_sync();
#pragma unroll 1
            for (int t = 0; t < 2; ++t) {
                const int nl = warp * 2 + t, n = node0 + nl;
                if (n >= n_end) break;
                float h[4], sum = 0.f, sq = 0.f;
#pragma unroll
                for (int k = 0; k < 4; ++k) { h[k] = sH[nl * 128 + lane + 32 * k]; sum += h[k]; sq = fmaf(h[k], h[k], sq); }
#pragma unroll
                for (int off = 16; off >= 1; off >>= 1) { sum += __shfl_xor_sync(0xffffffffu, sum, off); sq += __shfl_xor_sync(0xffffffffu, sq, off); }
                const float mean = sum * (1.0f / 128.0f);
                const float rstd = rsqrtf(fmaxf(sq * (1.0f / 128.0f) - mean * mean, 0.f) + 1e-6f);
                const float* fm = p.fin_mod + (size_t)sB[nl] * p.mod_stride;
                float o[6] = {0.f, 0.f, 0.f, 0.f, 0.f, 0.f};
#pragma unroll
                for (int k = 0; k < 4; ++k) {
                    const int c = lane + 32 * k;
                    const float tt = fmaf((h[k] - mean) * rstd, 1.0f + __ldg(fm + 128 + c), __ldg(fm + c));
                    const float2* w = reinterpret_cast<const float2*>(p.fin_w_t + c * 6);
                    const float2 w0 = __ldg(w), w1 = __ldg(w + 1), w2 = __ldg(w + 2);
                    o[0] = fmaf(tt, w0.x, o[0]); o[1] = fmaf(tt, w0.y, o[1]); o[2] = fmaf(tt, w1.x, o[2]);
                    o[3] = fmaf(tt, w1.y, o[3]); o[4] = fmaf(tt, w2.x, o[4]); o[5] = fmaf(tt, w2.y, o[5]);
                }
#pragma unroll
                for (int u = 0; u < 6; ++u) {
#pragma unroll
                    for (int off = 16; off >= 1; off >>= 1) o[u] += __shfl_xor_sync(0xffffffffu, o[u], off);
                    o[u] += __ldg(p.fin_b + u);
                }
                if (lane < 6) {
                    float mine = o[0];
#pragma unroll
                    for (int u = 1; u < 6; ++u) mine = lane == u ? o[u] : mine;
                    p.out6[(size_t)n * 6 + lane] = mine;
                }
                if (p.x_next != nullptr && lane < 3 && p.ddim) {
                    const float eps = lane == 0 ? o[0] : (lane == 1 ? o[1] : o[2]);
                    const float* nz = p.noise != nullptr ? p.noise + (size_t)n * 3 + lane : nullptr;
                    p.x_next[(size_t)n * 3 + lane] = ddim_update(p.x_t[(size_t)n * 3 + lane], eps, p.coef, nz);
                } else if (p.x_next != nullptr && lane < 3) {
                    const float eps = lane == 0 ? o[0] : (lane == 1 ? o[1] : o[2]);
                    const float vv = lane == 0 ? o[3] : (lane == 1 ? o[4] : o[5]);
                    const float x = p.x_t[(size_t)n * 3 + lane];
                    const float frac = (vv + 1.0f) / 2.0f;
                    const float logvar = frac * p.coef[1] + (1.0f - frac) * p.coef[0];
                    const float x0 = p.coef[2] * x - p.coef[3] * eps;
                    const float mean_ = p.coef[4] * x0 + p.coef[5] * x;
                    p.x_next[(size_t)n * 3 + lane] = mean_ + p.coef[6] * expf(0.5f * logvar) * p.noise[(size_t)n * 3 + lane];
                }
                if constexpr (INPAINT) {
                    if (lane < 3 && ir.keep[n]) {
                        const size_t k = (size_t)n * 3 + lane;
                        p.x_next[k] = inpaint_level(ir.level, ir.x0[k], ir.eps[k]);
                    }
                }
            }
        }
    }
    tc_fence_before();
    __syncthreads();
    if (tid == 0)
        for (int i = 0; i < N_BAR; ++i) asm volatile("mbarrier.inval.shared::cta.b64 [%0];" ::"r"(smem_u32(&sBar[i])) : "memory");
    __syncthreads();
}


}

void node_tc_update_params(Plan& p, int phase, const float* mod_base, int mod_stride_b, const float* x_t, const float* noise,
                           float* x_next, const float* coef_row, tc::NodeTcParams& np);

}
```

### codlad_b200/csrc/tc_common.cuh

```cuda
#pragma once
#include <cuda.h>
#include <cuda_fp16.h>
#include <stdint.h>

#include <cstdlib>
#include <utility>

#include "common.cuh"

namespace cb2 {
namespace tc {

constexpr int TILE_BYTES = 128 * 128 * 2;
constexpr int HALF_BYTES = TILE_BYTES / 2;
constexpr uint32_t SPIN_LIMIT = 1u << 22;

__device__ __forceinline__ uint32_t smem_u32(const void* p) { return (uint32_t)__cvta_generic_to_shared(p); }

__device__ __forceinline__ void mbar_init(uint32_t bar, uint32_t count) {
    asm volatile("mbarrier.init.shared::cta.b64 [%0], %1;" ::"r"(bar), "r"(count));
}
__device__ __forceinline__ void mbar_expect_tx(uint32_t bar, uint32_t bytes) {
    asm volatile("mbarrier.arrive.expect_tx.shared::cta.b64 _, [%0], %1;" ::"r"(bar), "r"(bytes) : "memory");
}
static __device__ unsigned int* g_trap_log = nullptr;
static __device__ __noinline__ void mbar_timeout(uint32_t bar, uint32_t parity, bool final) {
    if (g_trap_log != nullptr && blockIdx.x == g_trap_log[0] - 1u + (g_trap_log[0] == 0u ? blockIdx.x + 1u : 0u)) {
        const unsigned int claimed = atomicCAS(g_trap_log, 0u, blockIdx.x + 1u);
        if (claimed == 0u || claimed == blockIdx.x + 1u) {
            unsigned int* e = g_trap_log + 4 + (threadIdx.x >> 5) * 2;
            e[0] = bar; e[1] = (parity << 16) | (threadIdx.x & 0xffffu);
            __threadfence_system();
        }
    }
    if (final) __trap();
}
__device__ __forceinline__ bool mbar_try(uint32_t bar, uint32_t parity) {
    uint32_t done;
    asm volatile("{\n\t.reg .pred p;\n\tmbarrier.try_wait.parity.shared::cta.b64 p, [%1], %2;\n\tselp.u32 %0, 1, 0, p;\n\t}"
                 : "=r"(done) : "r"(bar), "r"(parity) : "memory");
    return done != 0;
}
static __device__ __noinline__ void mbar_wait_slow(uint32_t bar, uint32_t parity) {
    uint32_t spins = 0;
    while (true) {
        __nanosleep(64);
        if (mbar_try(bar, parity)) return;
        if (++spins == SPIN_LIMIT) mbar_timeout(bar, parity, false);
        if (spins > SPIN_LIMIT + (SPIN_LIMIT >> 1)) mbar_timeout(bar, parity, true);
    }
}
__device__ __forceinline__ void mbar_wait(uint32_t bar, uint32_t parity) {
    if (!mbar_try(bar, parity)) mbar_wait_slow(bar, parity);
}
__device__ __forceinline__ void tma_load_2d(uint32_t dst, const CUtensorMap* map, int c0, int c1, uint32_t bar) {
    asm volatile("cp.async.bulk.tensor.2d.shared::cluster.global.mbarrier::complete_tx::bytes [%0], [%1, {%2, %3}], [%4];"
                 ::"r"(dst), "l"(map), "r"(c0), "r"(c1), "r"(bar) : "memory");
}
__device__ __forceinline__ void tma_store_2d(const CUtensorMap* map, int c0, int c1, uint32_t src) {
    asm volatile("cp.async.bulk.tensor.2d.global.shared::cta.bulk_group [%0, {%1, %2}], [%3];"
                 ::"l"(map), "r"(c0), "r"(c1), "r"(src) : "memory");
}
__device__ __forceinline__ void tma_store_commit() { asm volatile("cp.async.bulk.commit_group;" ::: "memory"); }
__device__ __forceinline__ void tma_store_wait_read() { asm volatile("cp.async.bulk.wait_group.read 0;" ::: "memory"); }
__device__ __forceinline__ void tma_store_wait_all() { asm volatile("cp.async.bulk.wait_group 0;" ::: "memory"); }
__device__ __forceinline__ void fence_async_smem() { asm volatile("fence.proxy.async.shared::cta;" ::: "memory"); }
__device__ __forceinline__ void tc_fence_before() { asm volatile("tcgen05.fence::before_thread_sync;" ::: "memory"); }
__device__ __forceinline__ void tc_fence_after() { asm volatile("tcgen05.fence::after_thread_sync;" ::: "memory"); }

__device__ __forceinline__ uint64_t umma_desc(uint32_t addr, uint32_t lbo_bytes, uint32_t sbo_bytes) {
    return (uint64_t)((addr & 0x3FFFFu) >> 4) | ((uint64_t)(lbo_bytes >> 4) << 16) | ((uint64_t)(sbo_bytes >> 4) << 32) |
           (1ull << 46) | (2ull << 61);
}
__device__ __forceinline__ constexpr uint32_t umma_idesc(int M, int N, int a_mn, int b_mn) {
    return (1u << 4) | ((uint32_t)a_mn << 15) | ((uint32_t)b_mn << 16) | ((uint32_t)(N >> 3) << 17) | ((uint32_t)(M >> 4) << 24);
}
__device__ __forceinline__ void umma_f16(uint32_t tmem_d, uint64_t a, uint64_t b, uint32_t idesc, uint32_t accumulate) {
    asm volatile("{\n\t.reg .pred p;\n\tsetp.ne.b32 p, %4, 0;\n\ttcgen05.mma.cta_group::1.kind::f16 [%0], %1, %2, %3, p;\n\t}"
                 ::"r"(tmem_d), "l"(a), "l"(b), "r"(idesc), "r"(accumulate) : "memory");
}
__device__ __forceinline__ bool elect_one() {
    uint32_t pred;
    asm volatile("{\n\t.reg .pred p;\n\telect.sync _|p, 0xffffffff;\n\tselp.u32 %0, 1, 0, p;\n\t}" : "=r"(pred));
    return pred != 0;
}
__device__ __forceinline__ void umma_commit(uint32_t bar) {
    asm volatile("tcgen05.commit.cta_group::1.mbarrier::arrive::one.shared::cluster.b64 [%0];" ::"r"(bar) : "memory");
}
__device__ __forceinline__ void tmem_ld16(uint32_t taddr, float (&v)[16]) {
    uint32_t r[16];
    asm volatile("tcgen05.ld.sync.aligned.32x32b.x16.b32 {%0,%1,%2,%3,%4,%5,%6,%7,%8,%9,%10,%11,%12,%13,%14,%15}, [%16];"
                 : "=r"(r[0]), "=r"(r[1]), "=r"(r[2]), "=r"(r[3]), "=r"(r[4]), "=r"(r[5]), "=r"(r[6]), "=r"(r[7]), "=r"(r[8]), "=r"(r[9]),
                   "=r"(r[10]), "=r"(r[11]), "=r"(r[12]), "=r"(r[13]), "=r"(r[14]), "=r"(r[15])
                 : "r"(taddr));
    asm volatile("tcgen05.wait::ld.sync.aligned;" ::: "memory");
#pragma unroll
    for (int i = 0; i < 16; ++i) v[i] = __uint_as_float(r[i]);
}
__device__ __forceinline__ void tmem_ld16x2(uint32_t taddr, float (&v0)[16], float (&v1)[16]) {
    uint32_t r[32];
    asm volatile("tcgen05.ld.sync.aligned.32x32b.x16.b32 {%0,%1,%2,%3,%4,%5,%6,%7,%8,%9,%10,%11,%12,%13,%14,%15}, [%16];"
                 : "=r"(r[0]), "=r"(r[1]), "=r"(r[2]), "=r"(r[3]), "=r"(r[4]), "=r"(r[5]), "=r"(r[6]), "=r"(r[7]), "=r"(r[8]), "=r"(r[9]),
                   "=r"(r[10]), "=r"(r[11]), "=r"(r[12]), "=r"(r[13]), "=r"(r[14]), "=r"(r[15])
                 : "r"(taddr));
    asm volatile("tcgen05.ld.sync.aligned.32x32b.x16.b32 {%0,%1,%2,%3,%4,%5,%6,%7,%8,%9,%10,%11,%12,%13,%14,%15}, [%16];"
                 : "=r"(r[16]), "=r"(r[17]), "=r"(r[18]), "=r"(r[19]), "=r"(r[20]), "=r"(r[21]), "=r"(r[22]), "=r"(r[23]), "=r"(r[24]), "=r"(r[25]),
                   "=r"(r[26]), "=r"(r[27]), "=r"(r[28]), "=r"(r[29]), "=r"(r[30]), "=r"(r[31])
                 : "r"(taddr + 16u));
    asm volatile("tcgen05.wait::ld.sync.aligned;" ::: "memory");
#pragma unroll
    for (int i = 0; i < 16; ++i) { v0[i] = __uint_as_float(r[i]); v1[i] = __uint_as_float(r[16 + i]); }
}
__device__ __forceinline__ void tmem_st2(uint32_t taddr, float a, float b) {
    asm volatile("tcgen05.st.sync.aligned.32x32b.x2.b32 [%0], {%1, %2};" ::"r"(taddr), "r"(__float_as_uint(a)), "r"(__float_as_uint(b)) : "memory");
    asm volatile("tcgen05.wait::st.sync.aligned;" ::: "memory");
}
__device__ __forceinline__ void tmem_ld2_x4(uint32_t taddr, uint32_t col_stride, float (&v)[8]) {
    uint32_t r[8];
#pragma unroll
    for (int i = 0; i < 4; ++i)
        asm volatile("tcgen05.ld.sync.aligned.32x32b.x2.b32 {%0,%1}, [%2];" : "=r"(r[2 * i]), "=r"(r[2 * i + 1]) : "r"(taddr + i * col_stride));
    asm volatile("tcgen05.wait::ld.sync.aligned;" ::: "memory");
#pragma unroll
    for (int i = 0; i < 8; ++i) v[i] = __uint_as_float(r[i]);
}
__device__ __forceinline__ void tmem_ld8(uint32_t taddr, float (&v)[8]) {
    uint32_t r[8];
    asm volatile("tcgen05.ld.sync.aligned.32x32b.x8.b32 {%0,%1,%2,%3,%4,%5,%6,%7}, [%8];"
                 : "=r"(r[0]), "=r"(r[1]), "=r"(r[2]), "=r"(r[3]), "=r"(r[4]), "=r"(r[5]), "=r"(r[6]), "=r"(r[7]) : "r"(taddr));
    asm volatile("tcgen05.wait::ld.sync.aligned;" ::: "memory");
#pragma unroll
    for (int i = 0; i < 8; ++i) v[i] = __uint_as_float(r[i]);
}
__device__ __forceinline__ void tmem_ld4(uint32_t taddr, float (&v)[4]) {
    uint32_t r[4];
    asm volatile("tcgen05.ld.sync.aligned.32x32b.x4.b32 {%0,%1,%2,%3}, [%4];" : "=r"(r[0]), "=r"(r[1]), "=r"(r[2]), "=r"(r[3]) : "r"(taddr));
    asm volatile("tcgen05.wait::ld.sync.aligned;" ::: "memory");
#pragma unroll
    for (int i = 0; i < 4; ++i) v[i] = __uint_as_float(r[i]);
}
__device__ __forceinline__ void ldg256(const void* p, uint32_t (&r)[8]) {
    asm volatile("ld.global.nc.v8.b32 {%0,%1,%2,%3,%4,%5,%6,%7}, [%8];"
                 : "=r"(r[0]), "=r"(r[1]), "=r"(r[2]), "=r"(r[3]), "=r"(r[4]), "=r"(r[5]), "=r"(r[6]), "=r"(r[7]) : "l"(p));
}
__device__ __forceinline__ void ldg256_coherent(const void* p, uint32_t (&r)[8]) {
    asm volatile("ld.global.v8.b32 {%0,%1,%2,%3,%4,%5,%6,%7}, [%8];"
                 : "=r"(r[0]), "=r"(r[1]), "=r"(r[2]), "=r"(r[3]), "=r"(r[4]), "=r"(r[5]), "=r"(r[6]), "=r"(r[7]) : "l"(p) : "memory");
}
__device__ __forceinline__ float2 h2_to_f2(uint32_t u) {
    __half2 h = *reinterpret_cast<__half2*>(&u);
    return __half22float2(h);
}
__device__ __forceinline__ uint32_t f2_to_h2(float a, float b) {
    __half2 h = __floats2half2_rn(a, b);
    return *reinterpret_cast<uint32_t*>(&h);
}
__device__ __forceinline__ float gelu_fast(float x) {
    const float x2 = x * x;
    const float u = x * fmaf(x2, 0.03470094f, 0.80015698f);
    float t;
    asm("tanh.approx.f32 %0, %1;" : "=f"(t) : "f"(u));
    const float h = 0.5f * x;
    return fmaf(h, t, h);
}
__device__ __forceinline__ uint32_t tile_off(int r, int c16) {
    return (uint32_t)((c16 >> 3) * HALF_BYTES + r * 128 + (((c16 & 7) ^ (r & 7)) << 4));
}


__device__ __forceinline__ void mbar_arrive(uint32_t bar) {
    asm volatile("mbarrier.arrive.shared::cta.b64 _, [%0];" ::"r"(bar) : "memory");
}
__device__ __forceinline__ void stg256(void* p, const uint32_t (&r)[8]) {
    asm volatile("st.global.v8.b32 [%0], {%1,%2,%3,%4,%5,%6,%7,%8};"
                 ::"l"(p), "r"(r[0]), "r"(r[1]), "r"(r[2]), "r"(r[3]), "r"(r[4]), "r"(r[5]), "r"(r[6]), "r"(r[7]) : "memory");
}

__device__ __forceinline__ uint32_t pack_sat(float lo, float hi) {
    uint32_t d;
    asm("cvt.rn.satfinite.f16x2.f32 %0, %1, %2;" : "=r"(d) : "f"(hi), "f"(lo));
    return d;
}
__device__ __forceinline__ __half2 as_h2(uint32_t u) { return *reinterpret_cast<__half2*>(&u); }
__device__ __forceinline__ uint32_t as_u32(__half2 h) { return *reinterpret_cast<uint32_t*>(&h); }
__device__ __forceinline__ __half2 gelu2_h2(__half2 x) {
#ifdef CB2_X_NOMATH
    return x;
#endif
    const __half2 x2 = __hmul2(x, x);
    const __half2 pl = __hfma2(x2, __float2half2_rn(0.03470094f), __float2half2_rn(0.80015698f));
    const __half2 u = __hmul2(x, pl);
#ifdef CB2_X_NOTANH
    return __hfma2(x, u, x);
#endif
    uint32_t t;
    asm("tanh.approx.f16x2 %0, %1;" : "=r"(t) : "r"(as_u32(u)));
    return __hfma2(x, as_h2(t), x);
}


__device__ __forceinline__ void pdl_launch_dependents() { asm volatile("griddepcontrol.launch_dependents;" ::: "memory"); }
__device__ __forceinline__ void pdl_wait() { asm volatile("griddepcontrol.wait;" ::: "memory"); }

template <typename... KArgs, typename... Args>
inline cudaError_t launch_pdl(void (*kernel)(KArgs...), dim3 grid, dim3 block, size_t smem, cudaStream_t stream, Args&&... args) {
    cudaLaunchConfig_t cfg{};
    cfg.gridDim = grid; cfg.blockDim = block; cfg.dynamicSmemBytes = smem; cfg.stream = stream;
    static const bool no_pdl = getenv("CB2_NO_PDL") != nullptr;
    cudaLaunchAttribute attr[1];
    attr[0].id = cudaLaunchAttributeProgrammaticStreamSerialization;
    attr[0].val.programmaticStreamSerializationAllowed = no_pdl ? 0 : 1;
    cfg.attrs = attr; cfg.numAttrs = 1;
    return cudaLaunchKernelEx(&cfg, kernel, std::forward<Args>(args)...);
}

typedef CUresult (*EncodeTiledFn)(CUtensorMap*, CUtensorMapDataType, cuuint32_t, void*, const cuuint64_t*, const cuuint64_t*,
                                  const cuuint32_t*, const cuuint32_t*, CUtensorMapInterleave, CUtensorMapSwizzle,
                                  CUtensorMapL2promotion, CUtensorMapFloatOOBfill);

inline int encode_rows_map(EncodeTiledFn fn, CUtensorMap* map, const void* base, size_t rows, int box_rows) {
    const cuuint64_t gdim[2] = {128, (cuuint64_t)rows};
    const cuuint64_t gstride[1] = {256};
    const cuuint32_t box[2] = {64, (cuuint32_t)box_rows};
    const cuuint32_t estr[2] = {1, 1};
    CUresult r = fn(map, CU_TENSOR_MAP_DATA_TYPE_FLOAT16, 2, const_cast<void*>(base), gdim, gstride, box, estr,
                    CU_TENSOR_MAP_INTERLEAVE_NONE, CU_TENSOR_MAP_SWIZZLE_128B, CU_TENSOR_MAP_L2_PROMOTION_L2_256B,
                    CU_TENSOR_MAP_FLOAT_OOB_FILL_NONE);
    if (r != CUDA_SUCCESS) { set_error("cuTensorMapEncodeTiled failed (%d) rows=%zu box=%d", (int)r, rows, box_rows); return 1; }
    return 0;
}

inline int get_encode_fn(EncodeTiledFn* out) {
    void* fnp = nullptr;
    cudaDriverEntryPointQueryResult qres;
    CB2_CUDA(cudaGetDriverEntryPoint("cuTensorMapEncodeTiled", &fnp, cudaEnableDefault, &qres));
    if (!fnp || qres != cudaDriverEntryPointSuccess) { set_error("cuTensorMapEncodeTiled is not available in this driver"); return 1; }
    *out = reinterpret_cast<EncodeTiledFn>(fnp);
    return 0;
}

}

__device__ __forceinline__ void trace_window(unsigned long long* trace, int slot, bool end) {
    if (trace == nullptr) return;
    unsigned long long t;
    asm volatile("mov.u64 %0, %%globaltimer;" : "=l"(t));
    atomicMax(trace + 1024 + 2 * slot + (end ? 1 : 0), end ? t : ~t);
}

}
```

Measured before the change: 82480.

## Fold next-step node init into final update, stage weights in TMEM, adapt node tile

Folds the next sampling step's node_init (input projection plus first encoder projection) into the last node_update kernel, removing one launch per step. Weight tiles are now copied from shared memory into a TMEM ring with tcgen05.cp, and the MMAs read their A operand from TMEM. This needs an extra ring of barriers and more TMEM columns. The node kernel is templated on nodes per thread (6 or 8), choosing 6 when the graph is small relative to the SM count so more CTAs are launched. The risks are in barrier ordering for the ring and in the extra epilogue work added to the final update kernel.

```diff
diff --git a/codlad_b200/csrc/capi.cu b/codlad_b200/csrc/capi.cu
--- a/codlad_b200/csrc/capi.cu
+++ b/codlad_b200/csrc/capi.cu
@@ -487,20 +487,23 @@
 }
 
 int run_forward(Plan& p, const float* x, const float* mod_base, int mod_stride, const float* noise, float* x_next,
-                const float* coef_row, const float* inpaint_row, cudaStream_t s, int stop_after = -1) {
+                const float* coef_row, const float* inpaint_row, cudaStream_t s, int stop_after = -1, bool init_done = false,
+                bool fold_next = false) {
     int n = 0;
     auto done = [&]() { return stop_after >= 0 && ++n >= stop_after; };
     const bool tc = p.precision == PREC_F16 && p.node_tc != nullptr;
-    auto node_update = [&](int phase, const float* xt, const float* nz, float* xn, const float* cf, const float* iq) {
-        return tc ? launch_node_update_tc(p, phase, mod_base, mod_stride, xt, nz, xn, cf, iq, s)
+    auto node_update = [&](int phase, const float* xt, const float* nz, float* xn, const float* cf, const float* iq, bool fold) {
+        return tc ? launch_node_update_tc(p, phase, mod_base, mod_stride, xt, nz, xn, cf, iq, fold, s)
                   : launch_node_update(p, phase, mod_base, mod_stride, xt, nz, xn, cf, iq, s);
     };
-    if (int e = tc ? launch_node_init_tc(p, x, s) : launch_node_init(p, x, mod_base, mod_stride, s)) return e;
-    if (done()) return 0;
+    if (!init_done) {
+        if (int e = tc ? launch_node_init_tc(p, x, s) : launch_node_init(p, x, mod_base, mod_stride, s)) return e;
+        if (done()) return 0;
+    }
     for (int l = 0; l < 3; ++l) {
         if (int e = edge_dispatch(p, EDGE_ENC_NODE, l, mod_base, mod_stride, s)) return e;
         if (done()) return 0;
-        if (int e = node_update(l, nullptr, nullptr, nullptr, nullptr, nullptr)) return e;
+        if (int e = node_update(l, nullptr, nullptr, nullptr, nullptr, nullptr, false)) return e;
         if (done()) return 0;
         if (int e = edge_dispatch(p, EDGE_ENC_EDGE, l, mod_base, mod_stride, s)) return e;
         if (done()) return 0;
@@ -510,7 +513,7 @@
         if (done()) return 0;
         const bool last = l == 2;
         if (int e = node_update(3 + l, last ? x : nullptr, last ? noise : nullptr, last ? x_next : nullptr, last ? coef_row : nullptr,
-                                last ? inpaint_row : nullptr)) return e;
+                                last ? inpaint_row : nullptr, last && fold_next)) return e;
         if (done()) return 0;
     }
     return 0;
@@ -610,11 +613,13 @@
         p.launches++;
     }
     float *cur = h->xa, *nxt = h->xb;
+    const bool fold = p.precision == PREC_F16 && p.node_tc != nullptr;
     for (int step = p.coef_steps - 1; step >= 0; --step) {
         const float* mod_row = p.mod + (size_t)step * CB2_MOD_TOTAL;
         const float* step_noise = noise != nullptr ? noise + (size_t)step * n3 : nullptr;
         const float* inpaint_row = p.inpaint ? p.inp_coef + (size_t)step * 2 : nullptr;
-        if (int e = run_forward(p, cur, mod_row, 0, step_noise, nxt, p.coef + (size_t)step * 8, inpaint_row, s)) {
+        if (int e = run_forward(p, cur, mod_row, 0, step_noise, nxt, p.coef + (size_t)step * 8, inpaint_row, s, -1,
+                                fold && step < p.coef_steps - 1, fold && step > 0)) {
             char prev[1024];
             snprintf(prev, sizeof(prev), "%s", g_err);
             const unsigned int* tl = edge_tc_trap_log();
@@ -669,7 +674,8 @@
         p.graph_inpaint = p.inpaint;
     }
     CB2_CUDA(cudaGraphLaunch(p.graph, s));
-    p.launches += 16LL * p.coef_steps + (p.inpaint ? 1 : 0);
+    const bool fold = p.precision == PREC_F16 && p.node_tc != nullptr;
+    p.launches += (fold ? 15LL * p.coef_steps + 1 : 16LL * p.coef_steps) + (p.inpaint ? 1 : 0);
     return 0;
 }
 
@@ -787,7 +793,7 @@
             const bool last = layer == 5, tc = p.precision == PREC_F16 && p.node_tc != nullptr;
             const float *xt = last ? h->xa : nullptr, *nz = last ? h->xa : nullptr, *cf = last ? p.coef : nullptr;
             float* xn = last ? h->xb : nullptr;
-            return tc ? launch_node_update_tc(p, layer, p.mod, 0, xt, nz, xn, cf, nullptr, s)
+            return tc ? launch_node_update_tc(p, layer, p.mod, 0, xt, nz, xn, cf, nullptr, last, s)
                       : launch_node_update(p, layer, p.mod, 0, xt, nz, xn, cf, nullptr, s);
         }
         case 4: return launch_knn(p.X, p.lengths, p.F, p.L, p.K, p.nbr_dist, p.nbr_idx, s);
diff --git a/codlad_b200/csrc/model.h b/codlad_b200/csrc/model.h
--- a/codlad_b200/csrc/model.h
+++ b/codlad_b200/csrc/model.h
@@ -119,7 +119,7 @@
 void node_tc_release(Plan& p);
 int launch_node_init_tc(Plan& p, const float* x, cudaStream_t s);
 int launch_node_update_tc(Plan& p, int phase, const float* mod_base, int mod_stride_b, const float* x_t, const float* noise,
-                          float* x_next, const float* coef_row, const float* inpaint_row, cudaStream_t s);
+                          float* x_next, const float* coef_row, const float* inpaint_row, bool fold_init, cudaStream_t s);
 void edge_tc_release(Plan& p);
 const unsigned int* edge_tc_trap_log();
 
diff --git a/codlad_b200/csrc/node_tc.cu b/codlad_b200/csrc/node_tc.cu
--- a/codlad_b200/csrc/node_tc.cu
+++ b/codlad_b200/csrc/node_tc.cu
@@ -6,7 +6,7 @@
 
 namespace {
 
-template <bool INPAINT>
+template <bool INPAINT, int NPT>
 __device__ __forceinline__ void node_tc_run(const CUtensorMap& wmap, const NodeTcParams& p, const InpaintRows& ir) {
     extern __shared__ __align__(1024) unsigned char smem[];
     __shared__ uint32_t s_tmem;
@@ -22,28 +22,39 @@
     __syncthreads();
     tc_fence_after();
     const uint32_t tmem_base = s_tmem;
-    node_block<INPAINT>(smem, tmem_base, &wmap, p, blockIdx.x * NT, p.N, true, ir);
+    node_block<INPAINT, NPT>(smem, tmem_base, &wmap, p, blockIdx.x * 4 * NPT, p.N, true, ir);
     if (tid == 0) trace_window(p.trace, p.trace_slot, true);
     if (warp == 16) asm volatile("tcgen05.dealloc.cta_group::1.sync.aligned.b32 %0, 512;" ::"r"(tmem_base) : "memory");
 }
 
+template <int NPT>
 __global__ void __launch_bounds__(NODE_CTA_THREADS, 1) node_tc_kernel(const __grid_constant__ CUtensorMap wmap, const NodeTcParams p) {
-    node_tc_run<false>(wmap, p, InpaintRows{});
+    node_tc_run<false, NPT>(wmap, p, InpaintRows{});
 }
 
+template <int NPT>
 __global__ void __launch_bounds__(NODE_CTA_THREADS, 1) node_tc_inpaint_kernel(const __grid_constant__ CUtensorMap wmap, const NodeTcParams p,
                                                                              const __grid_constant__ InpaintRows ir) {
-    node_tc_run<true>(wmap, p, ir);
+    node_tc_run<true, NPT>(wmap, p, ir);
 }
 
 
-struct NodeTcState { CUtensorMap wmap; };
+struct NodeTcState {
+    CUtensorMap wmap;
+    int npt;
+};
+
+template <int NPT>
+int node_tc_launch_npt(const NodeTcState& st, const NodeTcParams& np, cudaStream_t s, const InpaintRows* ir) {
+    const dim3 grid((np.N + 4 * NPT - 1) / (4 * NPT)), block(NODE_CTA_THREADS);
+    if (ir != nullptr) CB2_CUDA(launch_pdl(node_tc_inpaint_kernel<NPT>, grid, block, NODE_TC_SMEM, s, st.wmap, np, *ir));
+    else CB2_CUDA(launch_pdl(node_tc_kernel<NPT>, grid, block, NODE_TC_SMEM, s, st.wmap, np));
+    return 0;
+}
 
 int node_tc_launch(Plan& p, NodeTcParams& np, cudaStream_t s, const InpaintRows* ir = nullptr) {
     const NodeTcState& st = *reinterpret_cast<const NodeTcState*>(p.node_tc);
-    const dim3 grid((np.N + NT - 1) / NT), block(NODE_CTA_THREADS);
-    if (ir != nullptr) CB2_CUDA(launch_pdl(node_tc_inpaint_kernel, grid, block, NODE_TC_SMEM, s, st.wmap, np, *ir));
-    else CB2_CUDA(launch_pdl(node_tc_kernel, grid, block, NODE_TC_SMEM, s, st.wmap, np));
+    if (int e = st.npt == 6 ? node_tc_launch_npt<6>(st, np, s, ir) : node_tc_launch_npt<8>(st, np, s, ir)) return e;
     CB2_LAUNCH_CHECK();
     p.launches++;
     return 0;
@@ -65,8 +76,12 @@
     NodeTcState* st = new NodeTcState();
     p.node_tc = st;
     if (encode_rows_map(fn, &st->wmap, p.model->dev_f16, (size_t)p.model->n_f16_blocks * 128, 128)) return 1;
-    CB2_CUDA(cudaFuncSetAttribute(node_tc_kernel, cudaFuncAttributeMaxDynamicSharedMemorySize, (int)NODE_TC_SMEM));
-    CB2_CUDA(cudaFuncSetAttribute(node_tc_inpaint_kernel, cudaFuncAttributeMaxDynamicSharedMemorySize, (int)NODE_TC_SMEM));
+    const long long N = (long long)p.NB * p.L;
+    st->npt = (N + 23) / 24 <= p.num_sms ? 6 : 8;
+    CB2_CUDA(cudaFuncSetAttribute(node_tc_kernel<8>, cudaFuncAttributeMaxDynamicSharedMemorySize, (int)NODE_TC_SMEM));
+    CB2_CUDA(cudaFuncSetAttribute(node_tc_inpaint_kernel<8>, cudaFuncAttributeMaxDynamicSharedMemorySize, (int)NODE_TC_SMEM));
+    CB2_CUDA(cudaFuncSetAttribute(node_tc_kernel<6>, cudaFuncAttributeMaxDynamicSharedMemorySize, (int)NODE_TC_SMEM));
+    CB2_CUDA(cudaFuncSetAttribute(node_tc_inpaint_kernel<6>, cudaFuncAttributeMaxDynamicSharedMemorySize, (int)NODE_TC_SMEM));
     return 0;
 }
 
@@ -88,7 +103,7 @@
 }
 
 void node_tc_update_params(Plan& p, int phase, const float* mod_base, int mod_stride_b, const float* x_t, const float* noise,
-                           float* x_next, const float* coef_row, tc::NodeTcParams& np) {
+                           float* x_next, const float* coef_row, bool fold_init, tc::NodeTcParams& np) {
     const DenoiserModel& m = *p.model;
     auto row_of = [&](const __half* w) { return (int)((w - m.dev_f16) / 128); };
     base_params(p, np);
@@ -129,14 +144,20 @@
             np.out6 = p.out6;
             np.x_t = x_t; np.noise = noise; np.x_next = x_next; np.coef = coef_row;
             np.ddim = p.update_kind == UPDATE_DDIM;
+            if (fold_init) {
+                np.fold_init = 1;
+                np.xin_w_t = m.xin_w_t; np.xin_b = m.xin_b;
+                np.n_proj = 1;
+                np.proj[0] = ProjTc{row_of(m.enc[0].W1a_h), row_of(m.enc[0].W1c_h), m.enc[0].b1, nullptr, p.P16[0], 0};
+            }
         }
     }
 }
 
 int launch_node_update_tc(Plan& p, int phase, const float* mod_base, int mod_stride_b, const float* x_t, const float* noise,
-                          float* x_next, const float* coef_row, const float* inpaint_row, cudaStream_t s) {
+                          float* x_next, const float* coef_row, const float* inpaint_row, bool fold_init, cudaStream_t s) {
     NodeTcParams np;
-    node_tc_update_params(p, phase, mod_base, mod_stride_b, x_t, noise, x_next, coef_row, np);
+    node_tc_update_params(p, phase, mod_base, mod_stride_b, x_t, noise, x_next, coef_row, fold_init && x_next != nullptr, np);
     if (inpaint_row != nullptr && np.do_final) {
         const InpaintRows ir{p.inp_keep, p.inp_x0, p.inp_eps, inpaint_row};
         return node_tc_launch(p, np, s, &ir);
diff --git a/codlad_b200/csrc/node_tc_body.cuh b/codlad_b200/csrc/node_tc_body.cuh
--- a/codlad_b200/csrc/node_tc_body.cuh
+++ b/codlad_b200/csrc/node_tc_body.cuh
@@ -32,6 +32,7 @@
     const float *x_t, *noise, *coef;
     float* x_next;
     int ddim;
+    int fold_init;
     unsigned long long* trace;
     int trace_slot;
 };
@@ -39,14 +40,14 @@
 constexpr int NODE_EPI_THREADS = 512;
 constexpr int NODE_CTA_THREADS = NODE_EPI_THREADS + 64;
 constexpr int NT = 32;
-constexpr int NPTH = NT / 4;
 constexpr int ACT_HALF = NT * 128;
 constexpr int ACT_BYTES = 2 * ACT_HALF;
 constexpr int N_SLOT = 5;
 constexpr int N_ACT = 6;
 constexpr int MAX_WT = 13;
 constexpr int R1 = 0, R2 = NT, R3 = 5 * NT;
-static_assert(NT == 32, "the LayerNorm transpose-reduce below is written for 8 nodes per thread");
+constexpr int RING = 6 * NT;
+static_assert(NT == 32, "the LayerNorm transpose-reduce below is written for at most 8 nodes per thread");
 
 __device__ __forceinline__ void node_epi_sync() { asm volatile("bar.sync 1, 512;" ::: "memory"); }
 __device__ __forceinline__ void node_group_sync(int cq) { asm volatile("bar.sync %0, 128;" ::"r"(cq + 2) : "memory"); }
@@ -67,10 +68,10 @@
     return n;
 }
 
-constexpr int N_BAR = 20;
+constexpr int N_BAR = 25;
 constexpr size_t NODE_TC_SMEM = (size_t)N_SLOT * TILE_BYTES + (size_t)N_ACT * ACT_BYTES + 2 * 4 * 4 * 16 * 4 + 4 * NT * 4 + N_BAR * 8 + 16;
 
-template <bool INPAINT>
+template <bool INPAINT, int NPT>
 __device__ __forceinline__ void node_block(unsigned char* smem, const uint32_t tmem_base, const CUtensorMap* wmap_p, const NodeTcParams& p,
                                            const int node0, const int n_end, const bool dep_wait, const InpaintRows& ir) {
     unsigned char* sW = smem;
@@ -82,14 +83,17 @@
     int* sZ = reinterpret_cast<int*>(sCnt + NT);
     uint64_t* sBar = reinterpret_cast<uint64_t*>(sZ + NT);
 
+    static_assert(NPT == 8 || NPT == 6, "nodes per epilogue thread");
+    constexpr int NB = 4 * NPT;
     const int tid = threadIdx.x, warp = tid >> 5, lane = tid & 31;
     auto bar_full = [&](int s) { return smem_u32(&sBar[s]); };
     auto bar_free = [&](int s) { return smem_u32(&sBar[N_SLOT + s]); };
     const uint32_t bar_mma = smem_u32(&sBar[10]), bar_act = smem_u32(&sBar[11]);
     auto bar_chunk = [&](int c) { return smem_u32(&sBar[12 + c]); };
     auto bar_mid = [&](int c) { return smem_u32(&sBar[16 + c]); };
+    auto bar_ring = [&](int s) { return smem_u32(&sBar[20 + s]); };
     if (tid == 0) {
-        for (int s = 0; s < N_SLOT; ++s) { mbar_init(bar_full(s), 1); mbar_init(bar_free(s), 1); }
+        for (int s = 0; s < N_SLOT; ++s) { mbar_init(bar_full(s), 1); mbar_init(bar_free(s), 1); mbar_init(bar_ring(s), 1); }
         mbar_init(bar_mma, 1); mbar_init(bar_act, NODE_EPI_THREADS / 32);
         for (int c = 0; c < 4; ++c) { mbar_init(bar_chunk(c), 1); mbar_init(bar_mid(c), NODE_EPI_THREADS / 32); }
         asm volatile("fence.mbarrier_init.release.cluster;" ::: "memory");
@@ -147,19 +151,37 @@
 #endif
             cmark(0);
             uint32_t ph_act = 0;
-            int ti = 0;
+            const int n_tiles = (p.do_update ? 9 : 0) + 2 * p.n_proj;
+            int ti = 0, n_staged = 0;
+            auto stage_upto = [&](int n, bool block) {
+#pragma unroll 1
+              for (n = min(n, n_tiles); n_staged < n; ++n_staged) {
+                const int i = n_staged, slot = i % N_SLOT, use = i / N_SLOT;
+                if (!block && !((use == 0 || mbar_try(bar_ring(slot), (uint32_t)((use - 1) & 1))) && mbar_try(bar_full(slot), (uint32_t)(use & 1))))
+                    break;
+                if (use > 0) mbar_wait(bar_ring(slot), (uint32_t)((use - 1) & 1));
+                mbar_wait(bar_full(slot), (uint32_t)(use & 1));
+                tc_fence_after();
+                const uint64_t a0 = umma_desc(smem_u32(sW + slot * TILE_BYTES), 16, 1024);
+                if (elect_one()) {
+#pragma unroll
+                    for (int k = 0; k < 8; ++k)
+                        tmem_cp_128x256b(tmem_base + (uint32_t)(RING + slot * 64 + k * 8), a0 + (uint64_t)(((k >> 2) * HALF_BYTES + (k & 3) * 32) >> 4));
+                    umma_commit(bar_free(slot));
+                }
+                __syncwarp();
+              }
+            };
             auto gemm = [&](int act, int d_col, bool accumulate) {
                 const int slot = ti % N_SLOT;
-                mbar_wait(bar_full(slot), (uint32_t)((ti / N_SLOT) & 1));
-                tc_fence_after();
                 cmark(6);
-                const uint64_t a0 = umma_desc(smem_u32(sW + slot * TILE_BYTES), 16, 1024), b0 = umma_desc(smem_u32(act_tile(act)), 16, 1024);
+                const uint64_t b0 = umma_desc(smem_u32(act_tile(act)), 16, 1024);
                 if (elect_one()) {
 #pragma unroll
                     for (int k = 0; k < 8; ++k)
-                        umma_f16(tmem_base + (uint32_t)d_col, a0 + (uint64_t)(((k >> 2) * HALF_BYTES + (k & 3) * 32) >> 4),
-                                 b0 + (uint64_t)(((k >> 2) * ACT_HALF + (k & 3) * 32) >> 4), IDESC, (accumulate || k > 0) ? 1u : 0u);
-                    umma_commit(bar_free(slot));
+                        umma_f16_tmem_a(tmem_base + (uint32_t)d_col, tmem_base + (uint32_t)(RING + slot * 64 + k * 8),
+                                        b0 + (uint64_t)(((k >> 2) * ACT_HALF + (k & 3) * 32) >> 4), IDESC, (accumulate || k > 0) ? 1u : 0u);
+                    umma_commit(bar_ring(slot));
                 }
                 __syncwarp();
                 cmark(7);
@@ -167,14 +189,23 @@
             };
             auto commit_phase = [&]() { if (elect_one()) umma_commit(bar_mma); __syncwarp(); cmark(4); };
             auto wait_act = [&]() { mbar_wait(bar_act, ph_act); ph_act ^= 1; tc_fence_after(); cmark(2); };
+            stage_upto(1, true);
+            stage_upto(N_SLOT, false);
             if (p.do_update) {
                 wait_act(); gemm(0, R1, false); commit_phase();
+                stage_upto(N_SLOT, true);
+                stage_upto(N_SLOT + 1, false);
                 wait_act();
                 for (int c = 0; c < 4; ++c) { gemm(1, R2 + c * NT, false); if (elect_one()) umma_commit(bar_chunk(c)); __syncwarp(); }
-                for (int c = 0; c < 4; ++c) { mbar_wait(bar_mid(c), 0); tc_fence_after(); cmark(8); gemm(2 + c, R3, c > 0); }
+                for (int c = 0; c < 4; ++c) {
+                    stage_upto(ti + 1, true); stage_upto(ti + 2, false);
+                    mbar_wait(bar_mid(c), 0); tc_fence_after(); cmark(8); gemm(2 + c, R3, c > 0);
+                }
                 commit_phase();
+                stage_upto(n_tiles, true);
             }
             if (p.n_proj > 0) {
+                stage_upto(n_tiles, true);
                 wait_act();
                 for (int j = 0; j < p.n_proj; ++j) {
                     gemm(0, R2 + (2 * j) * NT, false);
@@ -186,23 +217,26 @@
     } else {
         const int quarter = warp & 3, cq = warp >> 2;
         const int fl = quarter * 32 + lane;
-        const int nl0 = cq * NPTH;
+        const int nl0 = cq * NPT;
         const uint32_t tmem_lane = tmem_base + ((uint32_t)(quarter * 32) << 16) + (uint32_t)nl0;
         uint32_t ph_mma = 0;
-        int red_use = 0;
-        float v[NPTH];
+        float v[NPT];
+        auto ld_acc = [&](int col, float (&acc)[NPT]) {
+            if constexpr (NPT == 8) tmem_ld8(tmem_lane + (uint32_t)col, acc);
+            else tmem_ld2_x3(tmem_lane + (uint32_t)col, acc);
+        };
         auto publish = [&]() { fence_async_smem(); tc_fence_before(); __syncwarp(); if (lane == 0) mbar_arrive(bar_act); };
         auto wait_mma = [&]() { mbar_wait(bar_mma, ph_mma); ph_mma ^= 1; tc_fence_after(); };
         auto live = [&](int i) { return node0 + nl0 + i < n_end; };
         auto gnode = [&](int i) { return (size_t)(node0 + nl0 + i); };
         auto store_act = [&](unsigned char* tile, const float* x) {
 #pragma unroll
-            for (int i = 0; i < NPTH; ++i) sts_h(tile + act_off(nl0 + i, fl), __float2half_rn(x[i]));
-        };
-        auto node_stats = [&](float* mean, float* rstd) {
+            for (int i = 0; i < NPT; ++i) sts_h(tile + act_off(nl0 + i, fl), __float2half_rn(x[i]));
+        };
+        auto node_stats = [&](float* mean, float* rstd, int red_use) {
             float q[16];
 #pragma unroll
-            for (int i = 0; i < 8; ++i) { q[i] = v[i]; q[8 + i] = v[i] * v[i]; }
+            for (int i = 0; i < 8; ++i) { q[i] = i < NPT ? v[i] : 0.f; q[8 + i] = i < NPT ? v[i] * v[i] : 0.f; }
 #pragma unroll
             for (int cnt = 8, off = 16; cnt >= 1; cnt >>= 1, off >>= 1) {
                 const bool upper = (lane & off) != 0;
@@ -215,7 +249,7 @@
             }
             q[0] += __shfl_xor_sync(0xffffffffu, q[0], 1);
             const int idx = ((lane >> 4) & 1) * 8 + ((lane >> 3) & 1) * 4 + ((lane >> 2) & 1) * 2 + ((lane >> 1) & 1);
-            float* red = sRed + ((red_use & 1) * 16 + cq * 4) * 16;
+            float* red = sRed + (red_use * 16 + cq * 4) * 16;
             if ((lane & 1) == 0) red[quarter * 16 + idx] = q[0];
             node_group_sync(cq);
             float tot[16];
@@ -227,24 +261,23 @@
                 tot[k4 * 4 + 2] = (a.z + b.z) + (c.z + d.z); tot[k4 * 4 + 3] = (a.w + b.w) + (c.w + d.w);
             }
 #pragma unroll
-            for (int i = 0; i < 8; ++i) {
+            for (int i = 0; i < NPT; ++i) {
                 mean[i] = tot[i] * (1.0f / 128.0f);
                 rstd[i] = rsqrtf(fmaxf(tot[8 + i] * (1.0f / 128.0f) - mean[i] * mean[i], 0.f) + 1e-6f);
             }
-            ++red_use;
-        };
-        const int b_first = sB[nl0], b_last = sB[nl0 + NPTH - 1];
+        };
+        const int b_first = sB[nl0], b_last = sB[nl0 + NPT - 1];
         struct ModRow { float sh, sc, gt; };
         auto fetch_mod = [&](const float* mod_sh) {
             const float* m = mod_sh + (size_t)b_first * p.mod_stride + fl;
             return ModRow{__ldg(m), __ldg(m + 128), __ldg(m + 256)};
         };
         auto modulate = [&](const float* mod_sh, const ModRow& mr, bool masked) {
-            float mean[8], rstd[8];
-            node_stats(mean, rstd);
+            float mean[NPT], rstd[NPT];
+            node_stats(mean, rstd, masked ? 1 : 0);
             float A = mr.gt * (1.0f + mr.sc), Bv = mr.gt * mr.sh;
 #pragma unroll
-            for (int i = 0; i < 8; ++i) {
+            for (int i = 0; i < NPT; ++i) {
                 if (b_first != b_last) {
                     const float* m = mod_sh + (size_t)sB[nl0 + i] * p.mod_stride + fl;
                     const float sh = __ldg(m), sc = __ldg(m + 128), gt = __ldg(m + 256);
@@ -255,32 +288,44 @@
             }
         };
 
+        auto x_in = [&](const float* xs) {
+            const float w0 = __ldg(p.xin_w_t + fl), w1 = __ldg(p.xin_w_t + 128 + fl), w2 = __ldg(p.xin_w_t + 256 + fl), bb = __ldg(p.xin_b + fl);
+#pragma unroll
+            for (int i = 0; i < NPT; ++i) {
+                v[i] = 0.f;
+                if (live(i)) {
+                    const float* x = xs + gnode(i) * 3;
+                    v[i] = fmaf(x[2], w2, fmaf(x[1], w1, fmaf(x[0], w0, bb)));
+                }
+            }
+        };
+
         const int enc_mode = p.n_proj > 0 ? p.proj[p.n_proj - 1].add_enc : 0;
-        float pj_ba[2] = {0.f, 0.f}, pj_tab[NPTH], h_enc[NPTH];
+        float pj_ba[2] = {0.f, 0.f}, pj_tab[NPT], h_enc[NPT];
         int tab_j = -1;
 #pragma unroll
-        for (int i = 0; i < NPTH; ++i) { pj_tab[i] = 0.f; h_enc[i] = 0.f; }
+        for (int i = 0; i < NPT; ++i) { pj_tab[i] = 0.f; h_enc[i] = 0.f; }
 #pragma unroll
         for (int j = 0; j < 2; ++j) {
             if (j < p.n_proj) {
                 pj_ba[j] = __ldg(p.proj[j].ba + fl);
-                if (p.proj[j].table != nullptr) {
+                if (!INPAINT && p.proj[j].table != nullptr) {
                     tab_j = j;
 #pragma unroll
-                    for (int i = 0; i < NPTH; ++i) pj_tab[i] = __ldg(p.proj[j].table + sZ[nl0 + i] * 128 + fl);
+                    for (int i = 0; i < NPT; ++i) pj_tab[i] = __ldg(p.proj[j].table + sZ[nl0 + i] * 128 + fl);
                 }
             }
         }
         if (dep_wait) pdl_wait();
-        if (enc_mode == 1) {
-#pragma unroll
-            for (int i = 0; i < NPTH; ++i) h_enc[i] = live(i) ? p.hVenc[gnode(i) * 128 + fl] : 0.f;
+        if (!INPAINT && enc_mode == 1) {
+#pragma unroll
+            for (int i = 0; i < NPT; ++i) h_enc[i] = live(i) ? p.hVenc[gnode(i) * 128 + fl] : 0.f;
         }
         if (p.do_update) {
             {
                 const int node = tid >> 4, c16 = tid & 15;
                 uint32_t o[4] = {0u, 0u, 0u, 0u};
-                if (node0 + node < n_end) {
+                if (node < NB && node0 + node < n_end) {
                     uint32_t r8[8];
                     ldg256_coherent(p.S + (size_t)(node0 + node) * 128 + c16 * 8, r8);
 #pragma unroll
@@ -289,34 +334,32 @@
                 *reinterpret_cast<uint4*>(act_tile(0) + (c16 >> 3) * ACT_HALF + node * 128 + (((c16 & 7) ^ (node & 7)) << 4)) = make_uint4(o[0], o[1], o[2], o[3]);
             }
 #pragma unroll
-            for (int i = 0; i < NPTH; ++i) v[i] = live(i) ? p.hV[gnode(i) * 128 + fl] : 0.f;
+            for (int i = 0; i < NPT; ++i) v[i] = live(i) ? p.hV[gnode(i) * 128 + fl] : 0.f;
             publish();
             {
                 const float b3 = __ldg(p.b3 + fl);
                 const ModRow mr = fetch_mod(p.mod);
                 wait_mma();
-                float acc[8];
-                tmem_ld8(tmem_lane + R1, acc);
-#pragma unroll
-                for (int i = 0; i < NPTH; ++i) v[i] += (acc[i] + sCnt[nl0 + i] * b3) * (1.0f / 30.0f);
+                float acc[NPT];
+                ld_acc(R1, acc);
+#pragma unroll
+                for (int i = 0; i < NPT; ++i) v[i] += (acc[i] + sCnt[nl0 + i] * b3) * (1.0f / 30.0f);
                 modulate(p.mod, mr, false);
                 store_act(act_tile(1), v);
             }
             publish();
             {
-                float bi[4];
-#pragma unroll
-                for (int c = 0; c < 4; ++c) bi[c] = __ldg(p.bin + c * 128 + fl);
 #pragma unroll
                 for (int c = 0; c < 4; ++c) {
+                    const float bi = __ldg(p.bin + c * 128 + fl);
                     mbar_wait(bar_chunk(c), 0);
                     tc_fence_after();
-                    float acc[8];
-                    tmem_ld8(tmem_lane + (uint32_t)(R2 + c * NT), acc);
+                    float acc[NPT];
+                    ld_acc(R2 + c * NT, acc);
                     unsigned char* dst = act_tile(2 + c);
 #pragma unroll
-                    for (int j = 0; j < 4; ++j) {
-                        const __half2 g = gelu2_h2(as_h2(pack_sat(acc[2 * j] + bi[c], acc[2 * j + 1] + bi[c])));
+                    for (int j = 0; j < NPT / 2; ++j) {
+                        const __half2 g = gelu2_h2(as_h2(pack_sat(acc[2 * j] + bi, acc[2 * j + 1] + bi)));
                         sts_h(dst + act_off(nl0 + 2 * j, fl), __low2half(g));
                         sts_h(dst + act_off(nl0 + 2 * j + 1, fl), __high2half(g));
                     }
@@ -328,39 +371,30 @@
                 const float bo = __ldg(p.bout + fl);
                 const ModRow mr = fetch_mod(p.mod + 384);
                 wait_mma();
-                float acc[8];
-                tmem_ld8(tmem_lane + R3, acc);
-#pragma unroll
-                for (int i = 0; i < NPTH; ++i) v[i] += acc[i] + bo;
+                float acc[NPT];
+                ld_acc(R3, acc);
+#pragma unroll
+                for (int i = 0; i < NPT; ++i) v[i] += acc[i] + bo;
                 modulate(p.mod + 384, mr, true);
             }
         } else {
-            const float w0 = __ldg(p.xin_w_t + fl), w1 = __ldg(p.xin_w_t + 128 + fl), w2 = __ldg(p.xin_w_t + 256 + fl), bb = __ldg(p.xin_b + fl);
-#pragma unroll
-            for (int i = 0; i < NPTH; ++i) {
-                v[i] = 0.f;
-                if (live(i)) {
-                    const float* x = p.x + gnode(i) * 3;
-                    v[i] = fmaf(x[2], w2, fmaf(x[1], w1, fmaf(x[0], w0, bb)));
-                }
-            }
+            x_in(p.x);
         }
         auto write_state = [&]() {
 #pragma unroll
-            for (int i = 0; i < NPTH; ++i) {
+            for (int i = 0; i < NPT; ++i) {
                 if (live(i)) {
                     p.hV[gnode(i) * 128 + fl] = v[i];
                     if (p.write_enc) p.hVenc[gnode(i) * 128 + fl] = v[i];
                 }
             }
         };
-        if (p.n_proj == 0) write_state();
-        if (p.n_proj > 0) {
+        auto project = [&]() {
             store_act(act_tile(0), v);
             if (enc_mode) {
-                float hp[NPTH];
-#pragma unroll
-                for (int i = 0; i < NPTH; ++i)
+                float hp[NPT];
+#pragma unroll
+                for (int i = 0; i < NPT; ++i)
                     hp[i] = enc_mode == 1 ? (live(i) ? v[i] + h_enc[i] : 0.f) : 2.0f * v[i];
                 store_act(act_tile(1), hp);
             }
@@ -371,10 +405,10 @@
                 const ProjTc pj = p.proj[j];
 #pragma unroll
                 for (int which = 0; which < 2; ++which) {
-                    float acc[8];
-                    tmem_ld8(tmem_lane + (uint32_t)(R2 + (2 * j + which) * NT), acc);
-#pragma unroll
-                    for (int i = 0; i < NPTH; ++i) {
+                    float acc[NPT];
+                    ld_acc(R2 + (2 * j + which) * NT, acc);
+#pragma unroll
+                    for (int i = 0; i < NPT; ++i) {
                         if (live(i)) {
                             const float add = which == 0 ? (j == 0 ? pj_ba[0] : pj_ba[1]) : (j == tab_j ? pj_tab[i] : 0.f);
                             pj.out16[gnode(i) * 256 + which * 128 + fl] = __float2half_rn(acc[i] + add);
@@ -382,16 +416,18 @@
                     }
                 }
             }
-        }
+        };
+        if (p.n_proj == 0) write_state();
+        else if (!p.fold_init) project();
         if (p.do_final) {
             float* sH = reinterpret_cast<float*>(act_tile(2));
 #pragma unroll
-            for (int i = 0; i < NPTH; ++i) sH[(nl0 + i) * 128 + fl] = v[i];
+            for (int i = 0; i < NPT; ++i) sH[(nl0 + i) * 128 + fl] = v[i];
             node_epi_sync();
 #pragma unroll 1
             for (int t = 0; t < 2; ++t) {
                 const int nl = warp * 2 + t, n = node0 + nl;
-                if (n >= n_end) break;
+                if (nl >= NB || n >= n_end) break;
                 float h[4], sum = 0.f, sq = 0.f;
 #pragma unroll
                 for (int k = 0; k < 4; ++k) { h[k] = sH[nl * 128 + lane + 32 * k]; sum += h[k]; sq = fmaf(h[k], h[k], sq); }
@@ -443,6 +479,11 @@
                     }
                 }
             }
+            if (p.fold_init) {
+                node_epi_sync();
+                x_in(p.x_next);
+                project();
+            }
         }
     }
     tc_fence_before();
@@ -456,6 +497,6 @@
 }
 
 void node_tc_update_params(Plan& p, int phase, const float* mod_base, int mod_stride_b, const float* x_t, const float* noise,
-                           float* x_next, const float* coef_row, tc::NodeTcParams& np);
+                           float* x_next, const float* coef_row, bool fold_init, tc::NodeTcParams& np);
 
 }
diff --git a/codlad_b200/csrc/tc_common.cuh b/codlad_b200/csrc/tc_common.cuh
--- a/codlad_b200/csrc/tc_common.cuh
+++ b/codlad_b200/csrc/tc_common.cuh
@@ -79,6 +79,13 @@
     asm volatile("{\n\t.reg .pred p;\n\tsetp.ne.b32 p, %4, 0;\n\ttcgen05.mma.cta_group::1.kind::f16 [%0], %1, %2, %3, p;\n\t}"
                  ::"r"(tmem_d), "l"(a), "l"(b), "r"(idesc), "r"(accumulate) : "memory");
 }
+__device__ __forceinline__ void umma_f16_tmem_a(uint32_t tmem_d, uint32_t tmem_a, uint64_t b, uint32_t idesc, uint32_t accumulate) {
+    asm volatile("{\n\t.reg .pred p;\n\tsetp.ne.b32 p, %4, 0;\n\ttcgen05.mma.cta_group::1.kind::f16 [%0], [%1], %2, %3, p;\n\t}"
+                 ::"r"(tmem_d), "r"(tmem_a), "l"(b), "r"(idesc), "r"(accumulate) : "memory");
+}
+__device__ __forceinline__ void tmem_cp_128x256b(uint32_t taddr, uint64_t s) {
+    asm volatile("tcgen05.cp.cta_group::1.128x256b [%0], %1;" ::"r"(taddr), "l"(s) : "memory");
+}
 __device__ __forceinline__ bool elect_one() {
     uint32_t pred;
     asm volatile("{\n\t.reg .pred p;\n\telect.sync _|p, 0xffffffff;\n\tselp.u32 %0, 1, 0, p;\n\t}" : "=r"(pred));
@@ -123,6 +130,15 @@
     asm volatile("tcgen05.wait::ld.sync.aligned;" ::: "memory");
 #pragma unroll
     for (int i = 0; i < 8; ++i) v[i] = __uint_as_float(r[i]);
+}
+__device__ __forceinline__ void tmem_ld2_x3(uint32_t taddr, float (&v)[6]) {
+    uint32_t r[6];
+#pragma unroll
+    for (int i = 0; i < 3; ++i)
+        asm volatile("tcgen05.ld.sync.aligned.32x32b.x2.b32 {%0,%1}, [%2];" : "=r"(r[2 * i]), "=r"(r[2 * i + 1]) : "r"(taddr + 2 * i));
+    asm volatile("tcgen05.wait::ld.sync.aligned;" ::: "memory");
+#pragma unroll
+    for (int i = 0; i < 6; ++i) v[i] = __uint_as_float(r[i]);
 }
 __device__ __forceinline__ void tmem_ld8(uint32_t taddr, float (&v)[8]) {
     uint32_t r[8];
```

Result: slower. 81480 (median of 6 runs) (-1.2%).
